# elasticdeeplearning/edl

Measured on AMD Instinct MI355X. Metric: img/s, higher is better.
Workload: dtype bf16; 1 GPU; model=resnet50_vd, global_batch=32, parallelism=dp1, graph_capture=True

## Files before the change

edl_amd/csrc/common.h:

```cpp
#pragma once
#include <hip/hip_runtime.h>
#include <hip/hip_bf16.h>

constexpr int kWave = 64;

static inline int elementwise_grid(long long n, int block) {
  long long want = (n + block - 1) / block;
  long long cap = 256LL * 8;
  return (int)(want < cap ? want : cap);
}

__device__ __forceinline__ int xcd_swizzle(int orig, int nwg) {
  const int nx = 8;
  const int q = nwg / nx, r = nwg % nx;
  const int xcd = orig % nx, local = orig / nx;
  return (xcd < r ? xcd * (q + 1) : r * (q + 1) + (xcd - r) * q) + local;
}

__device__ __forceinline__ float wave_reduce_sum(float v) {
#pragma unroll
  for (int off = 32; off > 0; off >>= 1) v += __shfl_down(v, off, 64);
  return v;
}

__device__ __forceinline__ float wave_reduce_max(float v) {
#pragma unroll
  for (int off = 32; off > 0; off >>= 1) v = fmaxf(v, __shfl_down(v, off, 64));
  return v;
}
```

edl_amd/csrc/fused_adam.hip:

```cpp
#include "common.h"
#include "launchers.h"

namespace {

struct AdamCoef {
  float lr, b1, b2, omb1, omb2, eps, scale, step_size, sqrt_bc2;
  bool decoupled;
};

__device__ __forceinline__ void adam_elem(const AdamCoef& c, const float wd,
                                          const float g, float& p, float& m,
                                          float& v) {
  float gs = c.scale * g;
  if (c.decoupled)
    p *= 1.0f - c.lr * wd;
  else
    gs = fmaf(wd, p, gs);
  m = fmaf(c.b1, m, c.omb1 * gs);
  v = fmaf(c.b2, v, (c.omb2 * gs) * gs);
  const float denom = sqrtf(v) / c.sqrt_bc2 + c.eps;
  p = fmaf(-c.step_size, m / denom, p);
}

__device__ __forceinline__ int adam_find_seg(const int* s_end, int lo,
                                             const int nseg, const int e) {
  int hi = nseg - 1;
  while (lo < hi) {
    const int mid = (lo + hi) >> 1;
    if (s_end[mid] > e) hi = mid; else lo = mid + 1;
  }
  return lo;
}

__device__ __forceinline__ int adam_next_seg(const int* s_end, int s,
                                             const int nseg, const int e) {
  while (s + 1 < nseg && e >= s_end[s]) ++s;
  return s;
}

}

extern "C" __global__ void fused_adam_f32(
    float* __restrict__ p, const float* __restrict__ g, float* __restrict__ m,
    float* __restrict__ v, const int* __restrict__ step_dev,
    const float* __restrict__ lr_dev, const float lr_host, const float b1,
    const float b2, const float omb1, const float omb2, const float ln_b1,
    const float ln_b2, const float eps, const float wd, const float scale,
    const int decoupled, const long long n, const int* __restrict__ seg_end,
    const float* __restrict__ seg_wd, const int nseg) {
  extern __shared__ int s_tab[];
  int* s_end = s_tab;
  float* s_wd = reinterpret_cast<float*>(s_tab + nseg);
  if (nseg > 0) {
    for (int k = threadIdx.x; k < nseg; k += blockDim.x) {
      s_end[k] = seg_end[k];
      s_wd[k] = seg_wd[k];
    }
    __syncthreads();
  }

  AdamCoef c;
  c.lr = lr_dev ? *lr_dev : lr_host;
  const int t = *step_dev;
  const float tf = (float)(t > 1 ? t : 1);
  c.b1 = b1; c.b2 = b2; c.omb1 = omb1; c.omb2 = omb2;
  c.eps = eps; c.scale = scale; c.decoupled = decoupled != 0;
  c.step_size = c.lr / -expm1f(tf * ln_b1);
  c.sqrt_bc2 = sqrtf(-expm1f(tf * ln_b2));

  const long long n4 = n >> 2;
  const float4* g4 = reinterpret_cast<const float4*>(g);
  float4* p4 = reinterpret_cast<float4*>(p);
  float4* m4 = reinterpret_cast<float4*>(m);
  float4* v4 = reinterpret_cast<float4*>(v);
  long long i = (long long)blockIdx.x * blockDim.x + threadIdx.x;
  const long long stride = (long long)gridDim.x * blockDim.x;
  int s = 0;
  for (; i < n4; i += stride) {
    float4 pg = g4[i], pp = p4[i], pm = m4[i], pv = v4[i];
    float w0 = wd, w1 = wd, w2 = wd, w3 = wd;
    if (nseg > 0) {
      const int e = (int)(i << 2);
      s = adam_find_seg(s_end, s, nseg, e);
      int q = s;
      w0 = s_wd[q];
      q = adam_next_seg(s_end, q, nseg, e + 1);
      w1 = s_wd[q];
      q = adam_next_seg(s_end, q, nseg, e + 2);
      w2 = s_wd[q];
      q = adam_next_seg(s_end, q, nseg, e + 3);
      w3 = s_wd[q];
    }
    adam_elem(c, w0, pg.x, pp.x, pm.x, pv.x);
    adam_elem(c, w1, pg.y, pp.y, pm.y, pv.y);
    adam_elem(c, w2, pg.z, pp.z, pm.z, pv.z);
    adam_elem(c, w3, pg.w, pp.w, pm.w, pv.w);
    m4[i] = pm;
    v4[i] = pv;
    p4[i] = pp;
  }
  for (long long j = (n4 << 2) + (long long)blockIdx.x * blockDim.x + threadIdx.x;
       j < n; j += stride) {
    float w = wd;
    if (nseg > 0) w = s_wd[adam_find_seg(s_end, 0, nseg, (int)j)];
    float pj = p[j], mj = m[j], vj = v[j];
    adam_elem(c, w, g[j], pj, mj, vj);
    m[j] = mj;
    v[j] = vj;
    p[j] = pj;
  }
}

extern "C" void launch_fused_adam_f32(
    float* p, const float* g, float* m, float* v, const int* step_dev,
    const float* lr_dev, float lr, float b1, float b2, float omb1, float omb2,
    float ln_b1, float ln_b2, float eps, float wd, float scale, int decoupled,
    long long n, const int* seg_end, const float* seg_wd, int nseg,
    hipStream_t stream) {
  const int block = 256;
  const int grid = elementwise_grid((n + 3) / 4, block);
  const size_t lds = (size_t)nseg * (sizeof(int) + sizeof(float));
  hipLaunchKernelGGL(fused_adam_f32, dim3(grid), dim3(block), lds, stream, p,
                     g, m, v, step_dev, lr_dev, lr, b1, b2, omb1, omb2, ln_b1,
                     ln_b2, eps, wd, scale, decoupled, n, seg_end, seg_wd,
                     nseg);
}
```

edl_amd/csrc/fused_sgd.hip:

```cpp
#include "common.h"
#include "launchers.h"

extern "C" __global__ void fused_sgd_f32(
    float* __restrict__ p, const float* __restrict__ g, float* __restrict__ m,
    const float lr_host, const float mu, const float wd, const float scale,
    const long long n, const float* __restrict__ lr_dev) {
  const float lr = lr_dev ? *lr_dev : lr_host;
  const long long n4 = n >> 2;
  const float4* g4 = reinterpret_cast<const float4*>(g);
  float4* p4 = reinterpret_cast<float4*>(p);
  float4* m4 = reinterpret_cast<float4*>(m);
  long long i = (long long)blockIdx.x * blockDim.x + threadIdx.x;
  const long long stride = (long long)gridDim.x * blockDim.x;
  for (; i < n4; i += stride) {
    float4 pg = g4[i], pp = p4[i], pm = m4[i];
    float d0 = fmaf(scale, pg.x, wd * pp.x);
    float d1 = fmaf(scale, pg.y, wd * pp.y);
    float d2 = fmaf(scale, pg.z, wd * pp.z);
    float d3 = fmaf(scale, pg.w, wd * pp.w);
    pm.x = fmaf(mu, pm.x, d0);
    pm.y = fmaf(mu, pm.y, d1);
    pm.z = fmaf(mu, pm.z, d2);
    pm.w = fmaf(mu, pm.w, d3);
    pp.x = fmaf(-lr, pm.x, pp.x);
    pp.y = fmaf(-lr, pm.y, pp.y);
    pp.z = fmaf(-lr, pm.z, pp.z);
    pp.w = fmaf(-lr, pm.w, pp.w);
    m4[i] = pm;
    p4[i] = pp;
  }
  for (long long j = (n4 << 2) + (long long)blockIdx.x * blockDim.x + threadIdx.x;
       j < n; j += stride) {
    float d = fmaf(scale, g[j], wd * p[j]);
    float mv = fmaf(mu, m[j], d);
    m[j] = mv;
    p[j] = fmaf(-lr, mv, p[j]);
  }
}

extern "C" void launch_fused_sgd_f32(float* p, const float* g, float* m,
                                     float lr, float mu, float wd, float scale,
                                     long long n, const float* lr_dev,
                                     hipStream_t stream) {
  const int block = 256;
  const int grid = elementwise_grid((n + 3) / 4, block);
  hipLaunchKernelGGL(fused_sgd_f32, dim3(grid), dim3(block), 0, stream,
                     p, g, m, lr, mu, wd, scale, n, lr_dev);
}
```

edl_amd/csrc/launchers.h:

```cpp
#pragma once
#include <hip/hip_runtime_api.h>

constexpr int kStatsPartRowCap = 192;

extern "C" {

void launch_fused_sgd_f32(float* p, const float* g, float* m, float lr,
                          float mu, float wd, float scale, long long n,
                          const float* lr_dev, hipStream_t stream);

constexpr int kAdamMaxSegments = 1024;
void launch_fused_adam_f32(float* p, const float* g, float* m, float* v,
                           const int* step_dev, const float* lr_dev, float lr,
                           float b1, float b2, float omb1, float omb2,
                           float ln_b1, float ln_b2, float eps, float wd,
                           float scale, int decoupled, long long n,
                           const int* seg_end, const float* seg_wd, int nseg,
                           hipStream_t stream);

void launch_kd_ce_fwd_f32(const float* s, const float* t, float* lpr, int B,
                          int C, hipStream_t stream);
void launch_kd_ce_bwd_f32(const float* s, const float* t, float* ds,
                          float gob, int B, int C, hipStream_t stream);
void launch_kd_ce_fwd_bf16(const void* s, const void* t, float* lpr, int B,
                           int C, hipStream_t stream);
void launch_kd_ce_bwd_bf16(const void* s, const void* t, void* ds, float gob,
                           int B, int C, hipStream_t stream);

void launch_softmax_ce_fwd(const void* s, int is_bf16, const long long* ya,
                           const long long* yb, const float* lam,
                           float* loss_row, float* lse, int* rank, float eps,
                           int B, int C, hipStream_t stream);
void launch_softmax_ce_bwd(const void* s, int is_bf16, const float* lse,
                           const long long* ya, const long long* yb,
                           const float* lam, const float* gout, void* ds,
                           float eps, float inv_B, int B, int C,
                           hipStream_t stream);

int bn_stats_grid(long long M, int C);
int bn_bwd_grid(long long M, int C);
void launch_bn_stats(const void* x, float* partial, int grid, long long M,
                     int C, hipStream_t s);
void launch_bn_finalize(float* partial, int nblocks, int zero_src,
                        const float* gamma, const float* beta, float* mean,
                        float* invstd, float* scale, float* shift,
                        float* rmean, float* rvar, float momentum, float eps,
                        long long M, int C, hipStream_t s);
void launch_bn_apply(const void* x, const void* res, void* y,
                     unsigned char* mask, const float* scale,
                     const float* shift, long long M, int C, bool relu,
                     bool add, hipStream_t s);
void launch_bn_apply_pad(const void* x, void* yp, unsigned char* mask,
                         const float* scale, const float* shift, int Nimg,
                         int H, int W, int C, hipStream_t s);
void launch_bn_bwd_reduce(const void* dy, const unsigned char* mask,
                          const void* x, const float* mean,
                          const float* invstd, float* partial, int grid,
                          long long M, int C, bool relu, hipStream_t s);
void launch_bn_bwd_finalize(const float* partial, int nblocks, float* sums,
                            int C, float* db_acc, float* dg_acc,
                            hipStream_t s);
void launch_bn_bwd_dx(const void* dy, const unsigned char* mask,
                      const void* x, const float* mean, const float* invstd,
                      const float* gamma, const float* sums, void* dx,
                      void* dres, long long M, int C, bool relu, bool add,
                      bool training, hipStream_t s);
void launch_bn_bwd_dx_pad(const void* dy, const unsigned char* mask,
                          const void* x, const float* mean,
                          const float* invstd, const float* gamma,
                          const float* sums, void* dxp, int Nimg, int H,
                          int W, int C, bool relu, hipStream_t s);
void launch_bn_bwd_fused(const void* dy, const unsigned char* mask,
                         const void* x, const float* mean,
                         const float* invstd, const float* gamma,
                         float* partial, float* sums, float* db_acc,
                         float* dg_acc, void* dx, void* dres, int* ws,
                         int grid, int nfin, long long M, int C, bool relu,
                         bool add, hipStream_t s);

int gemm_bt_tiles_m(int M, int N);
void launch_gemm_bt(const void* A, const void* B, void* C, int M, int N,
                    int K, float* bn_part, hipStream_t s);
void launch_gemm_bt_splitk(const void* A, const void* B, float* Cf32, int M,
                           int N, int K, int splitk, hipStream_t s);

int conv3x3_tiles_m(int M, int Cout);
int conv3x3_small_tiles_m(int M);
int conv3x3_pick_splitk(int M, int Cout, int Cin);
void launch_pad_nhwc(const void* x, void* xp, int Nimg, int H, int W, int Hp,
                     int Wp, int C, hipStream_t s);
void launch_pad_nhwc_cpad(const void* x, void* xp, int Nimg, int H, int W,
                          int Hp, int Wp, int Creal, int Cpad,
                          hipStream_t s);
void launch_conv3x3(const void* xp, const void* w3, void* y, int M, int Cout,
                    int Cin, int HW_out, int W_out, int Hp, int Wp,
                    int stride, float* cpart, int splitk, float* bn_part,
                    hipStream_t s);
void launch_conv3x3_grouped(const void* xp, const void* w3g, void* y, int M,
                            int Cout, int Cin, int HW_out, int W_out, int Hp,
                            int Wp, int stride, int gw, hipStream_t s);
void launch_conv3x3_small(const void* xp, const void* w3s, void* y, int M,
                          int Cout_real, int cpt, int HW_out, int W_out,
                          int Hp, int Wp, int stride, float* bn_part,
                          hipStream_t s);
void launch_conv3x3s2_dgrad(const void* dyp, const void* wcat, void* dx,
                            int Nimg, int H, int W, int Cin, int Cout,
                            int Hop, int Wop, hipStream_t s);

void launch_gemm_tn_splitk(const void* A, const void* B, float* C, int N1,
                           int N2, int K, int splitk, hipStream_t s);
void launch_gemm_tn3x3_splitk(const void* dy, const void* xpad, float* C,
                              int Cout, int Cin, int M, int Ho, int Wo,
                              int Hp, int Wp, int stride, int splitk,
                              int perm, hipStream_t s);
void launch_gemm_tn3x3_splitk_apad(const void* dyp, const void* xpad,
                                   float* C, int Cout, int Cin, int M, int Ho,
                                   int Wo, int Hp, int Wp, int stride,
                                   int splitk, int perm, hipStream_t s);
void launch_gemm_tn3x3_small(const void* dy, const void* xpad, float* C,
                             int N1v, int N2v, int M, int Ho, int Wo, int Hp,
                             int Wp, int CinP, int stride, int splitk,
                             hipStream_t s);

void launch_transpose_pad(const void* in, void* out, int M, int C, int Mp,
                          hipStream_t s);
void launch_shift9_transpose(const void* xp, void* out, int M, int C, int Mp,
                             int HW_out, int W_out, int Hp, int Wp,
                             int stride, hipStream_t s);
void launch_repack_dgrad_w3(const void* in, void* out, int Co, int Ci,
                            int mode, hipStream_t s);
void launch_cast_bf16_zero(float* src, void* dst, long long n, hipStream_t s);

void launch_maxpool3x3s2_fwd(const void* x, void* y, unsigned char* idx,
                             int N, int H, int W, int Ho, int Wo, int C,
                             hipStream_t s);
void launch_maxpool3x3s2_bwd(const void* dy, const unsigned char* idx,
                             void* dx, int N, int H, int W, int Ho, int Wo,
                             int C, hipStream_t s);

void launch_avgpool2x2_fwd(const void* x, void* y, int N, int H, int W,
                           int Ho, int Wo, int C, hipStream_t s);
void launch_avgpool2x2_bwd(const void* dy, void* dx, int N, int H, int W,
                           int Ho, int Wo, int C, hipStream_t s);

int dgc_workspace_words();
void launch_dgc_accumulate(const float* g, float* u, float* v,
                           const float* p, float mu, float wd, long long n,
                           unsigned* ws, int hist_copies, hipStream_t stream);
void launch_dgc_hist(const float* v, long long n, unsigned* ws, int pass,
                     hipStream_t stream);
void launch_dgc_pick(unsigned* ws, int pass, unsigned k, hipStream_t stream);
void launch_dgc_compact(float* v, float* u, long long n, int* payload,
                        unsigned k, unsigned* ws, hipStream_t stream);
void launch_dgc_scatter_add(float* out, long long n, const int* payload,
                            long long k, hipStream_t stream);

}
```

edl_amd/csrc/module.cpp:

```cpp
#include <iterator>
#include <mutex>
#include <unordered_map>
#include <unordered_set>
#include <torch/extension.h>

#include <c10/hip/HIPStream.h>
#include <hip/hip_runtime.h>

#include "launchers.h"

namespace {

hipStream_t cur_stream() {
  return c10::hip::getCurrentHIPStream().stream();
}


void check_nhwc_bf16(const torch::Tensor& x, const char* who, int cmod = 0) {
  TORCH_CHECK(x.is_cuda() && x.dim() == 4 &&
                  x.scalar_type() == torch::kBFloat16 &&
                  x.is_contiguous(torch::MemoryFormat::ChannelsLast),
              who, ": 4-D channels_last bf16 GPU tensor required");
  TORCH_CHECK(cmod <= 0 || x.size(1) % cmod == 0, who, ": C % ", cmod);
}

int out_extent(int64_t in, int64_t stride) {
  return (int)((in - 1) / stride + 1);
}

int64_t auto_splitk(int tiles, int64_t upper) {
  const int64_t sk = std::max<int64_t>(1, 512 / std::max(1, tiles));
  return std::min(sk, upper);
}

void check_bt_operands(const torch::Tensor& a, const torch::Tensor& b,
                       const char* who) {
  TORCH_CHECK(a.is_cuda() && b.is_cuda() && a.dim() == 2 && b.dim() == 2 &&
                  a.size(1) == b.size(1),
              who, ": [M,K] x [N,K] GPU tensors required");
  TORCH_CHECK(a.scalar_type() == torch::kBFloat16 &&
                  b.scalar_type() == torch::kBFloat16,
              who, ": bf16 only");
  TORCH_CHECK(a.size(1) % 64 == 0 && b.size(0) % 64 == 0, who,
              ": K,N % 64 == 0");
}

int tn_tiles(int n) { return n / (n % 128 == 0 ? 128 : 64); }

torch::Tensor out_or_zeros(const c10::optional<torch::Tensor>& out,
                           int64_t rows, int64_t cols,
                           torch::TensorOptions opts, const char* msg) {
  if (!out.has_value())
    return torch::zeros({rows, cols}, opts.dtype(torch::kFloat32));
  TORCH_CHECK(out->is_contiguous() &&
                  out->scalar_type() == torch::kFloat32 &&
                  out->numel() == rows * cols,
              msg);
  return *out;
}

float* acc_ptr(const c10::optional<torch::Tensor>& acc, int64_t C,
               const char* msg) {
  if (!acc.has_value()) return nullptr;
  TORCH_CHECK(acc->numel() == C && acc->is_contiguous() &&
                  acc->scalar_type() == torch::kFloat32,
              msg);
  return acc->data_ptr<float>();
}

struct PadNHW {
  int64_t n = 0, h = 0, w = 0;
};

PadNHW parse_pad_hw(const std::vector<int64_t>& pad_hw, long long M,
                    const char* who) {
  TORCH_CHECK(pad_hw.size() == 2, who, ": pad_hw = (H, W)");
  PadNHW p;
  p.h = pad_hw[0];
  p.w = pad_hw[1];
  TORCH_CHECK(p.h >= 1 && p.w >= 1 && M >= 1 && M % (p.h * p.w) == 0, who,
              ": pad_hw does not divide the rows of x");
  p.n = M / (p.h * p.w);
  TORCH_CHECK(p.n * (p.h + 2) * (p.w + 2) < (1LL << 31), who,
              ": padded pixel count must stay below 2^31");
  return p;
}

void dgc_check_flat(const torch::Tensor& t, const char* name) {
  TORCH_CHECK(t.is_cuda() && t.scalar_type() == torch::kFloat32 &&
                  t.dim() == 1 && t.is_contiguous(),
              "dgc: ", name, " must be a flat contiguous fp32 GPU tensor");
  TORCH_CHECK(t.numel() >= 1 && t.numel() < (1LL << 31),
              "dgc: 1 <= n < 2^31 required for ", name);
}

unsigned* dgc_ws_ptr(const torch::Tensor& ws, const torch::Tensor& like) {
  TORCH_CHECK(ws.is_cuda() && ws.device() == like.device() &&
                  ws.scalar_type() == torch::kInt32 && ws.is_contiguous() &&
                  ws.numel() == dgc_workspace_words(),
              "dgc: workspace must be the int32 GPU tensor of "
              "dgc_workspace_words() zeros");
  return reinterpret_cast<unsigned*>(ws.data_ptr<int>());
}

void dgc_check_k(int64_t k, const torch::Tensor& v) {
  TORCH_CHECK(k >= 1 && k <= v.numel(), "dgc: 1 <= k <= n required");
}

int* dgc_payload_ptr(const torch::Tensor& payload, int64_t k,
                     const torch::Tensor& like) {
  TORCH_CHECK(payload.is_cuda() && payload.device() == like.device() &&
                  payload.scalar_type() == torch::kInt32 &&
                  payload.is_contiguous() && payload.dim() == 2 &&
                  payload.size(0) == 2 && payload.size(1) == k,
              "dgc: payload must be a contiguous int32 [2, k] GPU tensor");
  return payload.data_ptr<int>();
}

void dgc_accumulate(torch::Tensor g, torch::Tensor u, torch::Tensor v,
                    c10::optional<torch::Tensor> p, double mu, double wd,
                    torch::Tensor ws, int64_t hist_copies) {
  dgc_check_flat(g, "g");
  dgc_check_flat(u, "u");
  dgc_check_flat(v, "v");
  TORCH_CHECK(g.numel() == u.numel() && g.numel() == v.numel() &&
                  g.device() == u.device() && g.device() == v.device(),
              "dgc: g, u, v must match in size and device");
  const float* pp = nullptr;
  if (p.has_value()) {
    dgc_check_flat(*p, "p");
    TORCH_CHECK(p->numel() == g.numel() && p->device() == g.device(),
                "dgc: p must match g");
    pp = p->data_ptr<float>();
  }
  TORCH_CHECK(hist_copies == 1 || hist_copies == 4, "dgc: hist_copies 1 or 4");
  launch_dgc_accumulate(g.data_ptr<float>(), u.data_ptr<float>(),
                        v.data_ptr<float>(), pp, (float)mu, (float)wd,
                        (long long)g.numel(), dgc_ws_ptr(ws, g),
                        (int)hist_copies, cur_stream());
}

void dgc_hist(torch::Tensor v, torch::Tensor ws, int64_t pass) {
  dgc_check_flat(v, "v");
  TORCH_CHECK(pass == 1 || pass == 2, "dgc_hist: pass 1 or 2");
  launch_dgc_hist(v.data_ptr<float>(), (long long)v.numel(),
                  dgc_ws_ptr(ws, v), (int)pass, cur_stream());
}

void dgc_pick(torch::Tensor v, torch::Tensor ws, int64_t pass, int64_t k) {
  dgc_check_flat(v, "v");
  dgc_check_k(k, v);
  TORCH_CHECK(pass >= 0 && pass <= 2, "dgc_pick: pass 0..2");
  launch_dgc_pick(dgc_ws_ptr(ws, v), (int)pass, (unsigned)k, cur_stream());
}

void dgc_compact(torch::Tensor v, torch::Tensor u, torch::Tensor payload,
                 torch::Tensor ws) {
  dgc_check_flat(v, "v");
  dgc_check_flat(u, "u");
  TORCH_CHECK(u.numel() == v.numel() && u.device() == v.device(),
              "dgc: u must match v");
  const int64_t k = payload.dim() == 2 ? payload.size(1) : -1;
  dgc_check_k(k, v);
  launch_dgc_compact(v.data_ptr<float>(), u.data_ptr<float>(),
                     (long long)v.numel(), dgc_payload_ptr(payload, k, v),
                     (unsigned)k, dgc_ws_ptr(ws, v), cur_stream());
}

void dgc_select(torch::Tensor v, torch::Tensor u, torch::Tensor payload,
                torch::Tensor ws) {
  const int64_t k = payload.dim() == 2 ? payload.size(1) : -1;
  dgc_pick(v, ws, 0, k);
  dgc_hist(v, ws, 1);
  dgc_pick(v, ws, 1, k);
  dgc_hist(v, ws, 2);
  dgc_pick(v, ws, 2, k);
  dgc_compact(v, u, payload, ws);
}

void dgc_scatter_add(torch::Tensor out, torch::Tensor payload) {
  dgc_check_flat(out, "out");
  const int64_t k = payload.dim() == 2 ? payload.size(1) : -1;
  TORCH_CHECK(k >= 1, "dgc: payload must be int32 [2, k]");
  launch_dgc_scatter_add(out.data_ptr<float>(), (long long)out.numel(),
                         dgc_payload_ptr(payload, k, out), (long long)k,
                         cur_stream());
}

void fused_sgd(torch::Tensor p, torch::Tensor g, torch::Tensor m, double lr,
               double momentum, double weight_decay, double grad_scale,
               c10::optional<torch::Tensor> lr_dev) {
  TORCH_CHECK(p.is_cuda() && g.is_cuda() && m.is_cuda(), "fused_sgd: GPU tensors required");
  TORCH_CHECK(p.scalar_type() == torch::kFloat32 && g.scalar_type() == torch::kFloat32 &&
                  m.scalar_type() == torch::kFloat32,
              "fused_sgd: fp32 only");
  TORCH_CHECK(p.is_contiguous() && g.is_contiguous() && m.is_contiguous(),
              "fused_sgd: contiguous flat buffers required");
  TORCH_CHECK(p.numel() == g.numel() && p.numel() == m.numel(), "fused_sgd: size mismatch");
  const float* lrp = nullptr;
  if (lr_dev.has_value()) {
    TORCH_CHECK(lr_dev->is_cuda() && lr_dev->scalar_type() == torch::kFloat32 &&
                    lr_dev->numel() == 1,
                "fused_sgd: lr_dev must be a fp32 GPU scalar");
    lrp = lr_dev->data_ptr<float>();
  }
  launch_fused_sgd_f32(p.data_ptr<float>(), g.data_ptr<float>(), m.data_ptr<float>(),
                       (float)lr, (float)momentum, (float)weight_decay,
                       (float)grad_scale, (long long)p.numel(), lrp, cur_stream());
}


struct AdamTableSeen {
  c10::weak_intrusive_ptr<c10::TensorImpl> impl;
  uint32_t version;
  long long n;
};

void adam_check_table(const torch::Tensor& seg_end, long long n) {
  static std::mutex mu;
  static std::unordered_map<const c10::TensorImpl*, AdamTableSeen> seen;
  std::lock_guard<std::mutex> lock(mu);
  const c10::TensorImpl* key = seg_end.unsafeGetTensorImpl();
  const uint32_t version = seg_end._version();
  auto it = seen.find(key);
  if (it != seen.end() && !it->second.impl.expired() &&
      it->second.version == version && it->second.n == n)
    return;
  hipStreamCaptureStatus cap = hipStreamCaptureStatusNone;
  TORCH_CHECK(hipStreamIsCapturing(cur_stream(), &cap) == hipSuccess,
              "fused_adam: hipStreamIsCapturing failed");
  if (cap != hipStreamCaptureStatusNone) return;
  auto host = seg_end.cpu();
  const int* e = host.data_ptr<int>();
  int prev = 0;
  for (int64_t k = 0; k < host.numel(); ++k) {
    TORCH_CHECK(e[k] >= prev, "fused_adam: seg_end must not decrease");
    prev = e[k];
  }
  TORCH_CHECK(prev == n, "fused_adam: last seg_end (", prev,
              ") must equal numel (", n, ")");
  for (auto e = seen.begin(); e != seen.end();)
    e = e->second.impl.expired() ? seen.erase(e) : std::next(e);
  seen.insert_or_assign(
      key, AdamTableSeen{c10::weak_intrusive_ptr<c10::TensorImpl>(
                             seg_end.getIntrusivePtr()),
                         version, n});
}

void fused_adam(torch::Tensor p, torch::Tensor g, torch::Tensor m,
                torch::Tensor v, torch::Tensor step_dev, double lr,
                double beta1, double beta2, double eps, double weight_decay,
                double grad_scale, bool decoupled,
                c10::optional<torch::Tensor> lr_dev,
                c10::optional<torch::Tensor> seg_end,
                c10::optional<torch::Tensor> seg_wd) {
  TORCH_CHECK(p.is_cuda() && g.is_cuda() && m.is_cuda() && v.is_cuda(),
              "fused_adam: GPU tensors required");
  TORCH_CHECK(p.scalar_type() == torch::kFloat32 &&
                  g.scalar_type() == torch::kFloat32 &&
                  m.scalar_type() == torch::kFloat32 &&
                  v.scalar_type() == torch::kFloat32,
              "fused_adam: fp32 only");
  TORCH_CHECK(p.is_contiguous() && g.is_contiguous() && m.is_contiguous() &&
                  v.is_contiguous(),
              "fused_adam: contiguous flat buffers required");
  const long long n = p.numel();
  TORCH_CHECK(g.numel() == n && m.numel() == n && v.numel() == n,
              "fused_adam: size mismatch");
  TORCH_CHECK(g.device() == p.device() && m.device() == p.device() &&
                  v.device() == p.device(),
              "fused_adam: p, g, m, v must share a device");
  for (const torch::Tensor* t : {&p, &g, &m, &v})
    TORCH_CHECK(reinterpret_cast<uintptr_t>(t->data_ptr()) % 16 == 0,
                "fused_adam: p, g, m, v must be 16-byte aligned (float4)");
  TORCH_CHECK(step_dev.is_cuda() && step_dev.device() == p.device() &&
                  step_dev.scalar_type() == torch::kInt32 &&
                  step_dev.numel() == 1,
              "fused_adam: step_dev must be an int32 GPU scalar");
  TORCH_CHECK(beta1 >= 0.0 && beta1 < 1.0 && beta2 >= 0.0 && beta2 < 1.0,
              "fused_adam: betas must lie in [0, 1)");
  const float* lrp = nullptr;
  if (lr_dev.has_value()) {
    TORCH_CHECK(lr_dev->is_cuda() && lr_dev->device() == p.device() &&
                    lr_dev->scalar_type() == torch::kFloat32 &&
                    lr_dev->numel() == 1,
                "fused_adam: lr_dev must be a fp32 GPU scalar");
    lrp = lr_dev->data_ptr<float>();
  }
  const int* endp = nullptr;
  const float* wdp = nullptr;
  int nseg = 0;
  TORCH_CHECK(seg_end.has_value() == seg_wd.has_value(),
              "fused_adam: seg_end and seg_wd come together");
  if (seg_end.has_value()) {
    TORCH_CHECK(seg_end->is_cuda() && seg_wd->is_cuda() &&
                    seg_end->device() == p.device() &&
                    seg_wd->device() == p.device() &&
                    seg_end->scalar_type() == torch::kInt32 &&
                    seg_wd->scalar_type() == torch::kFloat32 &&
                    seg_end->is_contiguous() && seg_wd->is_contiguous() &&
                    seg_end->dim() == 1 && seg_wd->dim() == 1,
                "fused_adam: seg_end int32 / seg_wd fp32 flat GPU tensors");
    TORCH_CHECK(seg_end->numel() == seg_wd->numel(),
                "fused_adam: seg_end and seg_wd differ in length");
    TORCH_CHECK(seg_end->numel() >= 1 &&
                    seg_end->numel() <= kAdamMaxSegments,
                "fused_adam: 1 <= segments <= ", kAdamMaxSegments,
                " per bucket (got ", seg_end->numel(), ")");
    TORCH_CHECK(n < (1LL << 31),
                "fused_adam: a segment table needs numel < 2^31");
    adam_check_table(*seg_end, n);
    endp = seg_end->data_ptr<int>();
    wdp = seg_wd->data_ptr<float>();
    nseg = (int)seg_end->numel();
  }
  if (n == 0) return;
  launch_fused_adam_f32(
      p.data_ptr<float>(), g.data_ptr<float>(), m.data_ptr<float>(),
      v.data_ptr<float>(), step_dev.data_ptr<int>(), lrp, (float)lr,
      (float)beta1, (float)beta2, (float)(1.0 - beta1), (float)(1.0 - beta2),
      (float)std::log(beta1), (float)std::log(beta2), (float)eps,
      (float)weight_decay, (float)grad_scale, decoupled ? 1 : 0, n, endp, wdp,
      nseg, cur_stream());
}

torch::Tensor kd_ce_forward(torch::Tensor s, torch::Tensor t) {
  TORCH_CHECK(s.is_cuda() && t.is_cuda(), "kd_ce: GPU tensors required");
  TORCH_CHECK(s.dim() == 2 && t.sizes() == s.sizes(), "kd_ce: [B,C] logits expected");
  TORCH_CHECK(s.scalar_type() == t.scalar_type(), "kd_ce: dtype mismatch");
  auto sc = s.contiguous();
  auto tc = t.contiguous();
  const int B = (int)s.size(0), C = (int)s.size(1);
  auto lpr = torch::empty({B}, s.options().dtype(torch::kFloat32));
  if (s.scalar_type() == torch::kFloat32) {
    launch_kd_ce_fwd_f32(sc.data_ptr<float>(), tc.data_ptr<float>(),
                         lpr.data_ptr<float>(), B, C, cur_stream());
  } else if (s.scalar_type() == torch::kBFloat16) {
    launch_kd_ce_fwd_bf16(sc.data_ptr(), tc.data_ptr(), lpr.data_ptr<float>(), B, C,
                          cur_stream());
  } else {
    TORCH_CHECK(false, "kd_ce: fp32/bf16 only");
  }
  return lpr;
}

torch::Tensor kd_ce_backward(torch::Tensor s, torch::Tensor t, double gout_over_B) {
  auto sc = s.contiguous();
  auto tc = t.contiguous();
  const int B = (int)s.size(0), C = (int)s.size(1);
  auto ds = torch::empty_like(sc);
  if (s.scalar_type() == torch::kFloat32) {
    launch_kd_ce_bwd_f32(sc.data_ptr<float>(), tc.data_ptr<float>(), ds.data_ptr<float>(),
                         (float)gout_over_B, B, C, cur_stream());
  } else if (s.scalar_type() == torch::kBFloat16) {
    launch_kd_ce_bwd_bf16(sc.data_ptr(), tc.data_ptr(), ds.data_ptr(),
                          (float)gout_over_B, B, C, cur_stream());
  } else {
    TORCH_CHECK(false, "kd_ce: fp32/bf16 only");
  }
  return ds;
}

std::pair<const long long*, const float*> check_softmax_ce_inputs(
    const torch::Tensor& s, const torch::Tensor& ya,
    const c10::optional<torch::Tensor>& yb,
    const c10::optional<torch::Tensor>& lam) {
  TORCH_CHECK(s.is_cuda() && ya.device() == s.device(),
              "softmax_ce: logits and labels on one GPU required");
  TORCH_CHECK(s.dim() == 2 && s.size(0) >= 1 && s.size(1) >= 1,
              "softmax_ce: [B,C] logits expected");
  TORCH_CHECK(s.scalar_type() == torch::kFloat32 ||
                  s.scalar_type() == torch::kBFloat16,
              "softmax_ce: fp32/bf16 only");
  TORCH_CHECK(s.is_contiguous(), "softmax_ce: contiguous logits required");
  TORCH_CHECK(s.numel() < (1LL << 31), "softmax_ce: B*C < 2^31");
  const int64_t B = s.size(0);
  TORCH_CHECK(ya.scalar_type() == torch::kInt64 && ya.dim() == 1 &&
                  ya.numel() == B && ya.is_contiguous(),
              "softmax_ce: labels must be contiguous int64 [B]");
  TORCH_CHECK(yb.has_value() == lam.has_value(),
              "softmax_ce: labels_b and lam go together");
  if (!yb.has_value()) return {nullptr, nullptr};
  TORCH_CHECK(yb->is_cuda() && yb->scalar_type() == torch::kInt64 &&
                  yb->dim() == 1 && yb->numel() == B && yb->is_contiguous(),
              "softmax_ce: labels_b must be contiguous int64 [B] on the GPU");
  TORCH_CHECK(lam->is_cuda() && lam->scalar_type() == torch::kFloat32 &&
                  lam->dim() == 1 && lam->numel() == B && lam->is_contiguous(),
              "softmax_ce: lam must be contiguous fp32 [B] on the GPU");
  return {(const long long*)yb->data_ptr<int64_t>(), lam->data_ptr<float>()};
}

std::vector<torch::Tensor> softmax_ce_forward(torch::Tensor s, torch::Tensor ya,
                                              c10::optional<torch::Tensor> yb,
                                              c10::optional<torch::Tensor> lam,
                                              double eps) {
  auto mix = check_softmax_ce_inputs(s, ya, yb, lam);
  const int B = (int)s.size(0), C = (int)s.size(1);
  auto opts = s.options().dtype(torch::kFloat32);
  auto loss_row = torch::empty({B}, opts);
  auto lse = torch::empty({B}, opts);
  auto rank = torch::empty({B}, s.options().dtype(torch::kInt32));
  launch_softmax_ce_fwd(s.data_ptr(), s.scalar_type() == torch::kBFloat16,
                        (const long long*)ya.data_ptr<int64_t>(), mix.first,
                        mix.second, loss_row.data_ptr<float>(),
                        lse.data_ptr<float>(), rank.data_ptr<int>(), (float)eps,
                        B, C, cur_stream());
  return {loss_row, lse, rank};
}

torch::Tensor softmax_ce_backward(torch::Tensor s, torch::Tensor lse,
                                  torch::Tensor ya,
                                  c10::optional<torch::Tensor> yb,
                                  c10::optional<torch::Tensor> lam, double eps,
                                  torch::Tensor gout, double inv_B) {
  auto mix = check_softmax_ce_inputs(s, ya, yb, lam);
  const int B = (int)s.size(0), C = (int)s.size(1);
  TORCH_CHECK(lse.is_cuda() && lse.scalar_type() == torch::kFloat32 &&
                  lse.numel() == B && lse.is_contiguous(),
              "softmax_ce: lse must be contiguous fp32 [B] on the GPU");
  TORCH_CHECK(gout.is_cuda() && gout.scalar_type() == torch::kFloat32 &&
                  gout.numel() == 1,
              "softmax_ce: gout must be a fp32 GPU scalar");
  auto ds = torch::empty_like(s);
  launch_softmax_ce_bwd(s.data_ptr(), s.scalar_type() == torch::kBFloat16,
                        lse.data_ptr<float>(),
                        (const long long*)ya.data_ptr<int64_t>(), mix.first,
                        mix.second, gout.data_ptr<float>(), ds.data_ptr(),
                        (float)eps, (float)inv_B, B, C, cur_stream());
  return ds;
}

static std::unordered_set<const void*>& pooled_ptr_set() {
  static std::unordered_set<const void*> ptrs;
  return ptrs;
}

static torch::Tensor part_pool_get(int rows, int64_t cols,
                                   torch::TensorOptions opts) {
  static std::unordered_map<int64_t, torch::Tensor> pool;
  const int64_t key = ((int64_t)opts.device().index() << 48) |
                      ((int64_t)rows << 28) | cols;
  auto it = pool.find(key);
  if (it != pool.end()) return it->second;
  auto t = torch::zeros({rows, cols}, opts);
  pool.emplace(key, t);
  pooled_ptr_set().insert(t.data_ptr());
  return t;
}

torch::Tensor stats_part_buf(int tiles_m, int64_t cols,
                             torch::TensorOptions opts) {
  opts = opts.dtype(torch::kFloat32);
  const int rows = std::min(tiles_m, kStatsPartRowCap);
  return tiles_m > rows ? part_pool_get(rows, cols, opts)
                        : torch::empty({rows, cols}, opts);
}

void check_bn_inputs_eval(const torch::Tensor& x, int64_t C) {
  TORCH_CHECK(x.is_cuda() && x.scalar_type() == torch::kBFloat16,
              "bn: bf16 GPU tensor required");
  TORCH_CHECK(C % 8 == 0, "bn: C % 8 == 0 required, got ", C);
}

void check_bn_inputs(const torch::Tensor& x, int64_t C) {
  check_bn_inputs_eval(x, C);
  TORCH_CHECK(C <= 2048, "bn: C <= 2048 supported");
  TORCH_CHECK((C & (C - 1)) == 0,
              "bn: training needs a power-of-two C (8..2048): the stats and "
              "reduce kernels split each 256-thread block into C/8-thread "
              "rows; got ", C);
}

std::vector<torch::Tensor> bn_fwd_train(torch::Tensor x, torch::Tensor gamma,
                                        torch::Tensor beta, torch::Tensor rmean,
                                        torch::Tensor rvar, double momentum,
                                        double eps,
                                        c10::optional<torch::Tensor> res,
                                        bool relu,
                                        c10::optional<torch::Tensor> pre_part,
                                        c10::optional<std::vector<int64_t>> pad_hw) {
  const int64_t C = gamma.numel();
  TORCH_CHECK(x.dim() == 2 && x.size(1) == C && x.is_contiguous(),
              "bn: x must be a contiguous [M, C] view");
  check_bn_inputs(x, C);
  const long long M = x.numel() / C;
  PadNHW pad;
  if (pad_hw.has_value()) {
    TORCH_CHECK(relu && !res.has_value(),
                "bn: pad_hw needs relu and no residual");
    pad = parse_pad_hw(*pad_hw, M, "bn");
  }
  auto opts = gamma.options().dtype(torch::kFloat32);
  const int grid = bn_stats_grid(M, (int)C);
  auto partial = torch::empty({grid, 2 * C}, opts);
  auto mean = torch::empty({C}, opts);
  auto invstd = torch::empty({C}, opts);
  auto scale = torch::empty({C}, opts);
  auto shift = torch::empty({C}, opts);
  auto y = pad.n ? torch::empty({pad.n, pad.h + 2, pad.w + 2, C}, x.options())
                 : torch::empty_like(x);
  auto msk = relu ? torch::empty({M, C / 8}, x.options().dtype(torch::kUInt8))
                  : torch::empty({0}, x.options().dtype(torch::kUInt8));
  auto s = cur_stream();
  int fin_grid = grid;
  if (pre_part.has_value()) {
    TORCH_CHECK(pre_part->is_contiguous() &&
                    pre_part->scalar_type() == torch::kFloat32 &&
                    pre_part->dim() == 2 && pre_part->size(1) == 2 * C,
                "bn: pre_part [tiles, 2C] fp32");
    partial = *pre_part;
    fin_grid = (int)pre_part->size(0);
  } else {
    launch_bn_stats(x.data_ptr(), partial.data_ptr<float>(), grid, M, (int)C,
                    s);
  }
  const int zero_src =
      pre_part.has_value() &&
      pooled_ptr_set().count((const void*)partial.data_ptr());
  launch_bn_finalize(partial.data_ptr<float>(), fin_grid,
                     zero_src, gamma.data_ptr<float>(),
                     beta.data_ptr<float>(), mean.data_ptr<float>(),
                     invstd.data_ptr<float>(), scale.data_ptr<float>(),
                     shift.data_ptr<float>(),
                     rmean.defined() ? rmean.data_ptr<float>() : nullptr,
                     rvar.defined() ? rvar.data_ptr<float>() : nullptr,
                     (float)momentum, (float)eps, M, (int)C, s);
  if (pad.n) {
    launch_bn_apply_pad(x.data_ptr(), y.data_ptr(),
                        (unsigned char*)msk.data_ptr(),
                        scale.data_ptr<float>(), shift.data_ptr<float>(),
                        (int)pad.n, (int)pad.h, (int)pad.w, (int)C, s);
  } else {
    launch_bn_apply(x.data_ptr(), res.has_value() ? res->data_ptr() : nullptr,
                    y.data_ptr(),
                    relu ? (unsigned char*)msk.data_ptr() : nullptr,
                    scale.data_ptr<float>(), shift.data_ptr<float>(), M,
                    (int)C, relu, res.has_value(), s);
  }
  return {y, mean, invstd, msk};
}

torch::Tensor bn_fwd_eval(torch::Tensor x, torch::Tensor scale, torch::Tensor shift,
                          c10::optional<torch::Tensor> res, bool relu) {
  const int64_t C = scale.numel();
  check_bn_inputs_eval(x, C);
  const long long M = x.numel() / C;
  auto y = torch::empty_like(x);
  launch_bn_apply(x.data_ptr(), res.has_value() ? res->data_ptr() : nullptr,
                  y.data_ptr(), nullptr,
                  scale.data_ptr<float>(), shift.data_ptr<float>(),
                  M, (int)C, relu, res.has_value(), cur_stream());
  return y;
}

std::vector<torch::Tensor> bn_bwd(torch::Tensor dy, c10::optional<torch::Tensor> msk,
                                  torch::Tensor x,
                                  torch::Tensor mean, torch::Tensor invstd,
                                  torch::Tensor gamma, bool relu, bool add,
                                  bool training,
                                  c10::optional<torch::Tensor> dgamma_acc,
                                  c10::optional<torch::Tensor> dbeta_acc,
                                  c10::optional<std::vector<int64_t>> pad_hw) {
  const int64_t C = gamma.numel();
  check_bn_inputs(x, C);
  const long long M = x.numel() / C;
  auto opts = gamma.options().dtype(torch::kFloat32);
  const int grid = bn_bwd_grid(M, (int)C);
  auto sums = torch::empty({2, C}, opts);
  const char* fenv = getenv("EDL_BN_BWD_FUSED");
  const bool fused_bwd = fenv ? atoi(fenv) != 0 : false;
  PadNHW pad;
  if (pad_hw.has_value() && !(fused_bwd && training)) {
    TORCH_CHECK(training && !add, "bn_bwd: pad_hw needs training, no residual");
    pad = parse_pad_hw(*pad_hw, M, "bn_bwd");
  }
  auto dx = pad.n ? torch::empty({pad.n, pad.h + 2, pad.w + 2, C}, x.options())
                  : torch::empty_like(x);
  auto dres = add ? torch::empty_like(x) : torch::Tensor();
  auto s = cur_stream();
  auto dyc = dy.is_contiguous() ? dy : dy.contiguous();
  TORCH_CHECK(!relu || (msk.has_value() && msk->numel() == M * (C / 8)),
              "bn_bwd: relu path needs the fwd mask");
  const unsigned char* mp =
      relu ? (const unsigned char*)msk->data_ptr() : nullptr;
  float* dg_acc = acc_ptr(dgamma_acc, C, "bn_bwd: dgamma_acc fp32 [C]");
  float* db_acc = acc_ptr(dbeta_acc, C, "bn_bwd: dbeta_acc fp32 [C]");
  if (fused_bwd && training) {
    static std::unordered_map<int, torch::Tensor> ws_pool;
    const int dev = (int)x.device().index();
    auto wit = ws_pool.find(dev);
    if (wit == ws_pool.end())
      wit = ws_pool.emplace(dev, torch::zeros({4},
          x.options().dtype(torch::kInt32))).first;
    const long long total8 = M * (C / 8);
    int fgrid = (int)((total8 + 1023) / 1024);
    if (fgrid < grid) fgrid = grid;
    if (fgrid > 512) fgrid = 512;
    int nfin = (int)(2 * C) / 256;
    if (nfin < 1) nfin = 1;
    if (nfin > 8) nfin = 8;
    auto fpartial = torch::empty({fgrid, 2 * C}, opts);
    launch_bn_bwd_fused(dyc.data_ptr(), mp, x.data_ptr(),
                        mean.data_ptr<float>(), invstd.data_ptr<float>(),
                        gamma.data_ptr<float>(), fpartial.data_ptr<float>(),
                        sums.data_ptr<float>(), db_acc, dg_acc, dx.data_ptr(),
                        add ? dres.data_ptr() : nullptr,
                        wit->second.data_ptr<int>(), fgrid, nfin, M, (int)C,
                        relu, add, s);
    return {dx, sums[1], sums[0], dres};
  }
  auto partial = torch::empty({grid, 2 * C}, opts);
  launch_bn_bwd_reduce(dyc.data_ptr(), mp, x.data_ptr(),
                       mean.data_ptr<float>(), invstd.data_ptr<float>(),
                       partial.data_ptr<float>(), grid, M, (int)C, relu, s);
  launch_bn_bwd_finalize(partial.data_ptr<float>(), grid, sums.data_ptr<float>(),
                         (int)C, db_acc, dg_acc, s);
  if (pad.n) {
    launch_bn_bwd_dx_pad(dyc.data_ptr(), mp, x.data_ptr(),
                         mean.data_ptr<float>(), invstd.data_ptr<float>(),
                         gamma.data_ptr<float>(), sums.data_ptr<float>(),
                         dx.data_ptr(), (int)pad.n, (int)pad.h, (int)pad.w,
                         (int)C, relu, s);
  } else {
    launch_bn_bwd_dx(dyc.data_ptr(), mp, x.data_ptr(), mean.data_ptr<float>(),
                     invstd.data_ptr<float>(), gamma.data_ptr<float>(),
                     sums.data_ptr<float>(), dx.data_ptr(),
                     add ? dres.data_ptr() : nullptr, M, (int)C, relu, add,
                     training, s);
  }
  return {dx, sums[1], sums[0], dres};
}

std::vector<torch::Tensor> gemm_bt_impl(const torch::Tensor& a,
                                        const torch::Tensor& b,
                                        bool with_stats) {
  check_bt_operands(a, b, "gemm_bt");
  auto ac = a.contiguous();
  auto bc = b.contiguous();
  const int M = (int)a.size(0), K = (int)a.size(1), N = (int)b.size(0);
  auto c = torch::empty({M, N}, a.options());
  torch::Tensor part;
  if (with_stats)
    part = stats_part_buf(gemm_bt_tiles_m(M, N), 2 * N, a.options());
  launch_gemm_bt(ac.data_ptr(), bc.data_ptr(), c.data_ptr(), M, N, K,
                 with_stats ? part.data_ptr<float>() : nullptr, cur_stream());
  return {c, part};
}

torch::Tensor gemm_bt(torch::Tensor a, torch::Tensor b) {
  return gemm_bt_impl(a, b, false)[0];
}

std::vector<torch::Tensor> gemm_bt_stats(torch::Tensor a, torch::Tensor b) {
  return gemm_bt_impl(a, b, true);
}

torch::Tensor pad_nhwc_flat(const torch::Tensor& x, int cpad, hipStream_t s) {
  const int Nimg = (int)x.size(0), C = (int)x.size(1);
  const int H = (int)x.size(2), W = (int)x.size(3);
  const int Hp = H + 2, Wp = W + 2;
  auto xp = torch::empty({(long long)Nimg * Hp * Wp * cpad}, x.options());
  if (C == cpad) {
    launch_pad_nhwc(x.data_ptr(), xp.data_ptr(), Nimg, H, W, Hp, Wp, C, s);
  } else {
    launch_pad_nhwc_cpad(x.data_ptr(), xp.data_ptr(), Nimg, H, W, Hp, Wp, C,
                         cpad, s);
  }
  return xp;
}

torch::Tensor conv3x3_grouped_fwd(torch::Tensor x, torch::Tensor w3g,
                                  int64_t stride) {
  check_nhwc_bf16(x, "conv3x3g");
  const int Nimg = (int)x.size(0), Cin = (int)x.size(1);
  const int H = (int)x.size(2), W = (int)x.size(3);
  const int Cout = (int)w3g.size(0);
  TORCH_CHECK(w3g.size(1) % 9 == 0 && w3g.is_contiguous(), "conv3x3g: w3g");
  const int gw = (int)(w3g.size(1) / 9);
  TORCH_CHECK(gw % 64 == 0 && Cin % gw == 0, "conv3x3g: gw % 64, Cin % gw");
  TORCH_CHECK(Cin % 64 == 0 && Cout % 64 == 0 && Cin == Cout,
              "conv3x3g: C % 64, equal in/out");
  const int Hout = out_extent(H, stride), Wout = out_extent(W, stride);
  const long long M = (long long)Nimg * Hout * Wout;
  auto s = cur_stream();
  auto xp = pad_nhwc_flat(x, Cin, s);
  auto y = torch::empty({M, Cout}, x.options());
  launch_conv3x3_grouped(xp.data_ptr(), w3g.data_ptr(), y.data_ptr(), (int)M,
                         Cout, Cin, Hout * Wout, Wout, H + 2, W + 2,
                         (int)stride, gw, s);
  return y;
}

std::vector<torch::Tensor> conv3x3_small_impl(const torch::Tensor& x,
                                              const torch::Tensor& w3s,
                                              int64_t cout_real, int64_t cpt,
                                              int64_t stride,
                                              bool with_stats) {
  check_nhwc_bf16(x, "conv3x3s");
  TORCH_CHECK(stride == 1 || stride == 2, "conv3x3s: stride 1 or 2");
  TORCH_CHECK(cpt == 16 || cpt == 32 || cpt == 64, "conv3x3s: cpt 16/32/64");
  const int Nimg = (int)x.size(0), Cin = (int)x.size(1);
  const int H = (int)x.size(2), W = (int)x.size(3);
  TORCH_CHECK(Cin <= cpt, "conv3x3s: Cin <= cpt");
  const int taps_pad = cpt == 16 ? 12 : (cpt == 32 ? 10 : 9);
  TORCH_CHECK(w3s.is_contiguous() && w3s.size(0) == 64 &&
                  w3s.size(1) == taps_pad * cpt,
              "conv3x3s: w3s [64, taps_pad*cpt]");
  TORCH_CHECK(cout_real >= 1 && cout_real <= 64, "conv3x3s: cout <= 64");
  const int Hout = out_extent(H, stride), Wout = out_extent(W, stride);
  const long long M = (long long)Nimg * Hout * Wout;
  auto s = cur_stream();
  auto xp = pad_nhwc_flat(x, (int)cpt, s);
  auto y = torch::empty({M, cout_real}, x.options());
  torch::Tensor bpart;
  if (with_stats)
    bpart = stats_part_buf(conv3x3_small_tiles_m((int)M), 2 * cout_real,
                           x.options());
  launch_conv3x3_small(xp.data_ptr(), w3s.data_ptr(), y.data_ptr(), (int)M,
                       (int)cout_real, (int)cpt, Hout * Wout, Wout, H + 2,
                       W + 2, (int)stride,
                       with_stats ? bpart.data_ptr<float>() : nullptr, s);
  return {y, bpart};
}

torch::Tensor conv3x3_small_fwd(torch::Tensor x, torch::Tensor w3s,
                                int64_t cout_real, int64_t cpt,
                                int64_t stride) {
  return conv3x3_small_impl(x, w3s, cout_real, cpt, stride, false)[0];
}

std::vector<torch::Tensor> conv3x3_small_fwd_stats(torch::Tensor x,
                                                   torch::Tensor w3s,
                                                   int64_t cout_real,
                                                   int64_t cpt,
                                                   int64_t stride) {
  return conv3x3_small_impl(x, w3s, cout_real, cpt, stride, true);
}


torch::Tensor pad_nhwc(torch::Tensor x) {
  check_nhwc_bf16(x, "pad_nhwc", 8);
  const int Nimg = (int)x.size(0), C = (int)x.size(1);
  const int H = (int)x.size(2), W = (int)x.size(3);
  auto xp = torch::empty({Nimg, H + 2, W + 2, C}, x.options());
  launch_pad_nhwc(x.data_ptr(), xp.data_ptr(), Nimg, H, W, H + 2, W + 2, C,
                  cur_stream());
  return xp;
}

void check_padded(const torch::Tensor& xp, int64_t H, int64_t W,
                  const char* who) {
  TORCH_CHECK(xp.is_cuda() && xp.dim() == 4 &&
                  xp.scalar_type() == torch::kBFloat16 && xp.is_contiguous(),
              who, ": xp must be a contiguous [N, H+2, W+2, C] bf16 buffer");
  TORCH_CHECK(H >= 1 && W >= 1 && xp.size(1) == H + 2 && xp.size(2) == W + 2,
              who, ": xp is not the padded layout of an H x W image");
}

torch::Tensor conv3x3s2_dgrad_padded(torch::Tensor dyp, torch::Tensor wcat,
                                     int64_t H, int64_t W) {
  const int64_t Ho = (H + 1) / 2, Wo = (W + 1) / 2;
  check_padded(dyp, Ho, Wo, "s2dgrad");
  const int Nimg = (int)dyp.size(0), Cout = (int)dyp.size(3);
  const int Cin = (int)(wcat.size(0));
  TORCH_CHECK(wcat.is_contiguous() && wcat.size(1) == 9 * Cout,
              "s2dgrad: wcat [Cin, 9*Cout]");
  TORCH_CHECK(Cin % 64 == 0 && Cout % 64 == 0, "s2dgrad: C % 64");
  auto dx = torch::empty({(long long)Nimg * H * W, Cin}, dyp.options());
  launch_conv3x3s2_dgrad(dyp.data_ptr(), wcat.data_ptr(), dx.data_ptr(), Nimg,
                         (int)H, (int)W, Cin, Cout, (int)Ho + 2, (int)Wo + 2,
                         cur_stream());
  return dx;
}

torch::Tensor conv3x3s2_dgrad(torch::Tensor dy, torch::Tensor wcat,
                              int64_t H, int64_t W) {
  check_nhwc_bf16(dy, "s2dgrad dy", 64);
  TORCH_CHECK((H + 1) / 2 == dy.size(2) && (W + 1) / 2 == dy.size(3),
              "s2dgrad: shape");
  return conv3x3s2_dgrad_padded(pad_nhwc(dy), wcat, H, W);
}

torch::Tensor repack_dgrad_w3(torch::Tensor w_smaj, int64_t ci,
                              int64_t mode) {
  TORCH_CHECK(w_smaj.is_cuda() && w_smaj.scalar_type() == torch::kBFloat16 &&
                  w_smaj.is_contiguous() && w_smaj.dim() == 2 &&
                  w_smaj.size(1) == 9 * ci,
              "repack_dgrad_w3: [Co, 9*Ci] bf16");
  const int Co = (int)w_smaj.size(0);
  TORCH_CHECK(Co % 64 == 0 && ci % 64 == 0, "repack_dgrad_w3: C % 64");
  auto out = torch::empty({ci, (long long)9 * Co}, w_smaj.options());
  launch_repack_dgrad_w3(w_smaj.data_ptr(), out.data_ptr(), Co, (int)ci,
                         (int)mode, cur_stream());
  return out;
}

std::vector<torch::Tensor> maxpool3x3s2_fwd(torch::Tensor x) {
  check_nhwc_bf16(x, "maxpool3x3s2", 8);
  const int N = (int)x.size(0), C = (int)x.size(1);
  const int H = (int)x.size(2), W = (int)x.size(3);
  const int Ho = (H + 1) / 2, Wo = (W + 1) / 2;
  auto y = torch::empty({N, C, Ho, Wo},
                        x.options().memory_format(torch::MemoryFormat::ChannelsLast));
  auto idx = torch::empty({(long long)N * Ho * Wo * C},
                          x.options().dtype(torch::kUInt8));
  launch_maxpool3x3s2_fwd(x.data_ptr(), y.data_ptr(),
                          idx.data_ptr<unsigned char>(), N, H, W, Ho, Wo, C,
                          cur_stream());
  return {y, idx};
}

torch::Tensor maxpool3x3s2_bwd(torch::Tensor dy, torch::Tensor idx,
                               int64_t H, int64_t W) {
  check_nhwc_bf16(dy, "maxpool3x3s2_bwd");
  const int N = (int)dy.size(0), C = (int)dy.size(1);
  const int Ho = (int)dy.size(2), Wo = (int)dy.size(3);
  auto dx = torch::empty({N, C, (long long)H, (long long)W},
                         dy.options().memory_format(torch::MemoryFormat::ChannelsLast));
  launch_maxpool3x3s2_bwd(dy.data_ptr(), idx.data_ptr<unsigned char>(),
                          dx.data_ptr(), N, (int)H, (int)W, Ho, Wo, C,
                          cur_stream());
  return dx;
}

torch::Tensor avgpool2x2_fwd(torch::Tensor x) {
  check_nhwc_bf16(x, "avgpool2x2", 8);
  const int N = (int)x.size(0), C = (int)x.size(1);
  const int H = (int)x.size(2), W = (int)x.size(3);
  const int Ho = (H + 1) / 2, Wo = (W + 1) / 2;
  auto y = torch::empty({N, C, Ho, Wo},
                        x.options().memory_format(torch::MemoryFormat::ChannelsLast));
  launch_avgpool2x2_fwd(x.data_ptr(), y.data_ptr(), N, H, W, Ho, Wo, C,
                        cur_stream());
  return y;
}

torch::Tensor avgpool2x2_bwd(torch::Tensor dy, int64_t H, int64_t W) {
  const int N = (int)dy.size(0), C = (int)dy.size(1);
  const int Ho = (int)dy.size(2), Wo = (int)dy.size(3);
  auto dyc = dy.contiguous(torch::MemoryFormat::ChannelsLast);
  auto dx = torch::empty({N, C, H, W},
                         dy.options().memory_format(torch::MemoryFormat::ChannelsLast));
  launch_avgpool2x2_bwd(dyc.data_ptr(), dx.data_ptr(), N, (int)H, (int)W, Ho,
                        Wo, C, cur_stream());
  return dx;
}

torch::Tensor conv3x3_wgrad_operand_padded(torch::Tensor xp, int64_t H,
                                           int64_t W, int64_t stride) {
  check_padded(xp, H, W, "wgrad_operand");
  TORCH_CHECK(stride == 1 || stride == 2, "wgrad_operand: stride 1 or 2");
  const int Nimg = (int)xp.size(0), Cin = (int)xp.size(3);
  const int Hp = (int)H + 2, Wp = (int)W + 2;
  const int Hout = out_extent(H, stride), Wout = out_extent(W, stride);
  const int M = Nimg * Hout * Wout;
  const int Mp = (M + 63) / 64 * 64;
  auto out = torch::empty({(long long)9 * Cin, Mp}, xp.options());
  launch_shift9_transpose(xp.data_ptr(), out.data_ptr(), M, Cin, Mp,
                          Hout * Wout, Wout, Hp, Wp, (int)stride,
                          cur_stream());
  return out;
}

torch::Tensor conv3x3_wgrad_operand(torch::Tensor x, int64_t stride) {
  auto xp = pad_nhwc(x);
  return conv3x3_wgrad_operand_padded(xp, x.size(2), x.size(3), stride);
}

torch::Tensor gemm_bt_splitk(torch::Tensor a, torch::Tensor b, int64_t splitk) {
  check_bt_operands(a, b, "gemm_bt_splitk");
  auto ac = a.contiguous();
  auto bc = b.contiguous();
  const int M = (int)a.size(0), K = (int)a.size(1), N = (int)b.size(0);
  if (splitk <= 0) {
    const int tiles = ((M + 127) / 128) * ((N + 63) / 64);
    splitk = auto_splitk(tiles, K / 64);
  }
  auto c = torch::zeros({M, N}, a.options().dtype(torch::kFloat32));
  launch_gemm_bt_splitk(ac.data_ptr(), bc.data_ptr(), c.data_ptr<float>(), M, N,
                        K, (int)splitk, cur_stream());
  return c;
}

torch::Tensor gemm_tn_splitk(torch::Tensor a, torch::Tensor b, int64_t splitk,
                             c10::optional<torch::Tensor> out) {
  TORCH_CHECK(a.is_cuda() && b.is_cuda() && a.dim() == 2 && b.dim() == 2 &&
                  a.size(0) == b.size(0),
              "gemm_tn_splitk: [K,N1] x [K,N2] GPU");
  TORCH_CHECK(a.scalar_type() == torch::kBFloat16 &&
                  b.scalar_type() == torch::kBFloat16,
              "gemm_tn_splitk: bf16 only");
  auto ac = a.contiguous();
  auto bc = b.contiguous();
  const int K = (int)a.size(0), N1 = (int)a.size(1), N2 = (int)b.size(1);
  TORCH_CHECK(N1 % 64 == 0 && N2 % 64 == 0, "gemm_tn_splitk: N1,N2 % 64");
  const int nchunks = (K + 63) / 64;
  if (splitk <= 0) splitk = auto_splitk(tn_tiles(N1) * tn_tiles(N2), nchunks);
  splitk = std::min<int64_t>(splitk, nchunks);
  auto c = out_or_zeros(out, N1, N2, a.options(),
                        "gemm_tn_splitk: out fp32 contiguous [N1,N2]");
  launch_gemm_tn_splitk(ac.data_ptr(), bc.data_ptr(), c.data_ptr<float>(), N1,
                        N2, K, (int)splitk, cur_stream());
  return c;
}

torch::Tensor gemm_tn3x3_splitk_padded(torch::Tensor dy, torch::Tensor xp,
                                       int64_t H64, int64_t W64,
                                       int64_t stride, int64_t splitk,
                                       c10::optional<torch::Tensor> out) {
  check_padded(xp, H64, W64, "gemm_tn3x3");
  TORCH_CHECK(stride == 1 || stride == 2, "gemm_tn3x3: stride 1 or 2");
  const bool dy_padded = dy.dim() == 4;
  TORCH_CHECK(dy.is_cuda() && (dy.dim() == 2 || dy_padded) &&
                  dy.scalar_type() == torch::kBFloat16,
              "gemm_tn3x3: dy [M,Cout] or padded [N,Ho+2,Wo+2,Cout] bf16");
  const int Nimg = (int)xp.size(0), Cin = (int)xp.size(3);
  const int H = (int)H64, W = (int)W64;
  const int Hp = H + 2, Wp = W + 2;
  const int Ho = out_extent(H, stride), Wo = out_extent(W, stride);
  const int M = Nimg * Ho * Wo;
  const int Cout = (int)dy.size(dy_padded ? 3 : 1);
  if (dy_padded) {
    check_padded(dy, Ho, Wo, "gemm_tn3x3 dy");
    TORCH_CHECK(dy.size(0) == Nimg, "gemm_tn3x3: dy batch != xp batch");
  } else {
    TORCH_CHECK((int)dy.size(0) == M, "gemm_tn3x3: dy2d rows != N*Ho*Wo");
  }
  TORCH_CHECK(Cin % 64 == 0 && Cout % 64 == 0, "gemm_tn3x3: C % 64");
  auto dyc = dy.contiguous();
  auto s = cur_stream();
  const int nchunks = (M + 63) / 64;
  if (splitk <= 0)
    splitk = auto_splitk(tn_tiles(Cout) * 9 * tn_tiles(Cin), nchunks);
  splitk = std::min<int64_t>(splitk, nchunks);
  auto c = out_or_zeros(out, Cout, 9 * Cin, xp.options(),
                        "gemm_tn3x3_splitk: out fp32 contiguous");
  const int perm = (c.dim() == 2 && c.size(1) == 9 * Cin) ? 0 : Cin;
  if (dy_padded)
    launch_gemm_tn3x3_splitk_apad(dyc.data_ptr(), xp.data_ptr(),
                                  c.data_ptr<float>(), Cout, Cin, M, Ho, Wo,
                                  Hp, Wp, (int)stride, (int)splitk, perm, s);
  else
    launch_gemm_tn3x3_splitk(dyc.data_ptr(), xp.data_ptr(),
                             c.data_ptr<float>(), Cout, Cin, M, Ho, Wo, Hp, Wp,
                             (int)stride, (int)splitk, perm, s);
  return c;
}

torch::Tensor gemm_tn3x3_splitk(torch::Tensor dy2d, torch::Tensor x,
                                int64_t stride, int64_t splitk,
                                c10::optional<torch::Tensor> out) {
  TORCH_CHECK(dy2d.dim() == 2, "gemm_tn3x3: dy2d [M,Cout] bf16");
  auto xp = pad_nhwc(x);
  return gemm_tn3x3_splitk_padded(dy2d, xp, x.size(2), x.size(3), stride,
                                  splitk, out);
}

torch::Tensor transpose_pad(torch::Tensor x) {
  TORCH_CHECK(x.is_cuda() && x.dim() == 2 &&
                  x.scalar_type() == torch::kBFloat16 && x.is_contiguous(),
              "transpose_pad: contiguous 2-D bf16 GPU tensor");
  const int M = (int)x.size(0), C = (int)x.size(1);
  TORCH_CHECK(C % 8 == 0, "transpose_pad: C % 8");
  const int Mp = (M + 63) / 64 * 64;
  auto y = torch::empty({C, Mp}, x.options());
  launch_transpose_pad(x.data_ptr(), y.data_ptr(), M, C, Mp, cur_stream());
  return y;
}

struct Conv3x3Geom {
  int Cin, Cout, Hp, Wp, Hout, Wout;
  long long M;
};

Conv3x3Geom conv3x3_geom(const torch::Tensor& xp, const torch::Tensor& w3,
                         int64_t stride, int64_t H, int64_t W) {
  check_padded(xp, H, W, "conv3x3");
  TORCH_CHECK(stride == 1 || stride == 2, "conv3x3: stride 1 or 2");
  Conv3x3Geom g;
  g.Cin = (int)xp.size(3);
  g.Cout = (int)w3.size(0);
  TORCH_CHECK(w3.size(1) == 9 * g.Cin && w3.is_contiguous(),
              "conv3x3: w3 shape");
  TORCH_CHECK(g.Cin % 64 == 0 && g.Cout % 64 == 0, "conv3x3: C % 64");
  g.Hp = (int)H + 2;
  g.Wp = (int)W + 2;
  g.Hout = out_extent(H, stride);
  g.Wout = out_extent(W, stride);
  g.M = (long long)xp.size(0) * g.Hout * g.Wout;
  return g;
}

std::vector<torch::Tensor> conv3x3_fwd_impl(const torch::Tensor& xp,
                                            const torch::Tensor& w3,
                                            int64_t stride, int64_t H,
                                            int64_t W, bool with_stats) {
  const Conv3x3Geom g = conv3x3_geom(xp, w3, stride, H, W);
  const int M = (int)g.M;
  auto s = cur_stream();
  const int splitk = conv3x3_pick_splitk(M, g.Cout, g.Cin);
  torch::Tensor y, bpart;
  if (splitk > 1) {
    auto part =
        part_pool_get(M, g.Cout, xp.options().dtype(torch::kFloat32));
    launch_conv3x3(xp.data_ptr(), w3.data_ptr(), nullptr, M, g.Cout, g.Cin,
                   g.Hout * g.Wout, g.Wout, g.Hp, g.Wp, (int)stride,
                   part.data_ptr<float>(), splitk, nullptr, s);
    y = torch::empty({g.M, g.Cout}, xp.options());
    launch_cast_bf16_zero(part.data_ptr<float>(), y.data_ptr(),
                          g.M * g.Cout, s);
  } else {
    y = torch::empty({g.M, g.Cout}, xp.options());
    if (with_stats)
      bpart = stats_part_buf(conv3x3_tiles_m(M, g.Cout), 2 * g.Cout,
                             xp.options());
    launch_conv3x3(xp.data_ptr(), w3.data_ptr(), y.data_ptr(), M, g.Cout,
                   g.Cin, g.Hout * g.Wout, g.Wout, g.Hp, g.Wp, (int)stride,
                   nullptr, 1, with_stats ? bpart.data_ptr<float>() : nullptr,
                   s);
  }
  return {y, bpart};
}

torch::Tensor conv3x3_fwd_padded(torch::Tensor xp, torch::Tensor w3,
                                 int64_t stride, int64_t H, int64_t W) {
  return conv3x3_fwd_impl(xp, w3, stride, H, W, false)[0];
}

std::vector<torch::Tensor> conv3x3_fwd_stats_padded(torch::Tensor xp,
                                                    torch::Tensor w3,
                                                    int64_t stride, int64_t H,
                                                    int64_t W) {
  return conv3x3_fwd_impl(xp, w3, stride, H, W, true);
}

torch::Tensor conv3x3_fwd(torch::Tensor x, torch::Tensor w3, int64_t stride) {
  check_nhwc_bf16(x, "conv3x3", 64);
  return conv3x3_fwd_padded(pad_nhwc(x), w3, stride, x.size(2), x.size(3));
}

std::vector<torch::Tensor> conv3x3_fwd_stats(torch::Tensor x, torch::Tensor w3,
                                             int64_t stride) {
  check_nhwc_bf16(x, "conv3x3", 64);
  return conv3x3_fwd_stats_padded(pad_nhwc(x), w3, stride, x.size(2),
                                  x.size(3));
}

torch::Tensor gemm_tn3x3_small(torch::Tensor dy2d, torch::Tensor x,
                               int64_t stride, int64_t splitk) {
  check_nhwc_bf16(x, "tn3x3s");
  TORCH_CHECK(stride == 1 || stride == 2, "tn3x3s: stride 1 or 2");
  const int Nimg = (int)x.size(0), Cin = (int)x.size(1);
  const int H = (int)x.size(2), W = (int)x.size(3);
  TORCH_CHECK(Cin >= 1 && Cin <= 64, "tn3x3s: Cin <= 64");
  const int Hout = out_extent(H, stride), Wout = out_extent(W, stride);
  const long long M = (long long)Nimg * Hout * Wout;
  TORCH_CHECK(dy2d.is_cuda() && dy2d.is_contiguous() && dy2d.dim() == 2 &&
                  dy2d.scalar_type() == torch::kBFloat16 &&
                  dy2d.size(0) == M && dy2d.size(1) == 64,
              "tn3x3s: dy2d [M, 64] bf16");
  int CinP = 8;
  while (CinP < Cin) CinP <<= 1;
  const int N2 = 9 * CinP;
  const int N2v = (N2 + 63) / 64 * 64;
  auto s = cur_stream();
  auto xp = pad_nhwc_flat(x, CinP, s);
  if (splitk <= 0) {
    const int nch = (int)((M + 63) / 64);
    splitk = auto_splitk(N2v / 64, std::max(1, nch));
  }
  auto c = torch::zeros({64, N2v}, x.options().dtype(torch::kFloat32));
  launch_gemm_tn3x3_small(dy2d.data_ptr(), xp.data_ptr(), c.data_ptr<float>(),
                          64, N2v, (int)M, Hout, Wout, H + 2, W + 2, CinP,
                          (int)stride, (int)splitk, s);
  return c;
}

}

PYBIND11_MODULE(TORCH_EXTENSION_NAME, m) {
  m.def("fused_sgd", &fused_sgd,
        "fused flat momentum-SGD update (p,g,m flat fp32; folds grad_scale)",
        py::arg("p"), py::arg("g"), py::arg("m"), py::arg("lr"),
        py::arg("momentum"), py::arg("weight_decay"), py::arg("grad_scale"),
        py::arg("lr_dev") = py::none());
  m.def("fused_adam", &fused_adam,
        "fused flat Adam/AdamW update (p,g,m,v flat fp32; step count and lr "
        "read from device scalars; optional per-segment decay table of at "
        "most 1024 segments); does not advance step_dev",
        py::arg("p"), py::arg("g"), py::arg("m"), py::arg("v"),
        py::arg("step_dev"), py::arg("lr"), py::arg("beta1"),
        py::arg("beta2"), py::arg("eps"), py::arg("weight_decay"),
        py::arg("grad_scale"), py::arg("decoupled"),
        py::arg("lr_dev") = py::none(), py::arg("seg_end") = py::none(),
        py::arg("seg_wd") = py::none());
  m.attr("ADAM_MAX_SEGMENTS") = kAdamMaxSegments;
  m.def("dgc_workspace_words", &dgc_workspace_words,
        "int32 words of the (zero-initialised) DGC select workspace");
  m.def("dgc_accumulate", &dgc_accumulate,
        "DGC: u = mu*u + (g + wd*p); v += u; radix-select pass 0 histogram",
        py::arg("g"), py::arg("u"), py::arg("v"), py::arg("p"), py::arg("mu"),
        py::arg("wd"), py::arg("ws"), py::arg("hist_copies") = 4);
  m.def("dgc_hist", &dgc_hist, "DGC radix-select histogram pass 1 or 2",
        py::arg("v"), py::arg("ws"), py::arg("pass_"));
  m.def("dgc_pick", &dgc_pick, "DGC radix-select: fix one digit (pass 0..2)",
        py::arg("v"), py::arg("ws"), py::arg("pass_"), py::arg("k"));
  m.def("dgc_compact", &dgc_compact,
        "DGC: write the selected (idx, bits) into payload [2,k]; zero v, u",
        py::arg("v"), py::arg("u"), py::arg("payload"), py::arg("ws"));
  m.def("dgc_select", &dgc_select,
        "DGC: pick 0, (hist, pick) x 2 and compact, after dgc_accumulate",
        py::arg("v"), py::arg("u"), py::arg("payload"), py::arg("ws"));
  m.def("dgc_scatter_add", &dgc_scatter_add,
        "DGC decode: out[idx] += val for one rank's payload",
        py::arg("out"), py::arg("payload"));
  m.def("kd_ce_forward", &kd_ce_forward, "KD soft-label CE forward -> per-row loss");
  m.def("kd_ce_backward", &kd_ce_backward, "KD soft-label CE backward -> dlogits");
  m.def("softmax_ce_forward", &softmax_ce_forward,
        "hard-label CE (label smoothing, optional mixup) fwd -> "
        "(loss_row, lse, rank)",
        py::arg("s"), py::arg("labels"), py::arg("labels_b") = py::none(),
        py::arg("lam") = py::none(), py::arg("eps") = 0.0);
  m.def("softmax_ce_backward", &softmax_ce_backward,
        "hard-label CE bwd -> dlogits (gout is a device scalar)",
        py::arg("s"), py::arg("lse"), py::arg("labels"), py::arg("labels_b"),
        py::arg("lam"), py::arg("eps"), py::arg("gout"), py::arg("inv_B"));
  m.def("bn_fwd_train", &bn_fwd_train,
        "fused NHWC bf16 BN(+add)+ReLU train fwd -> (y, mean, invstd, mask)",
        py::arg("x"), py::arg("gamma"), py::arg("beta"), py::arg("rmean"),
        py::arg("rvar"), py::arg("momentum"), py::arg("eps"), py::arg("res"),
        py::arg("relu"), py::arg("pre_part") = py::none(),
        py::arg("pad_hw") = py::none());
  m.def("bn_fwd_eval", &bn_fwd_eval, "fused NHWC bf16 BN(+add)+ReLU eval fwd");
  m.def("bn_bwd", &bn_bwd,
        "fused BN(+add)+ReLU bwd -> (dx, dgamma, dbeta, dres?)",
        py::arg("dy"), py::arg("msk"), py::arg("x"), py::arg("mean"),
        py::arg("invstd"), py::arg("gamma"), py::arg("relu"), py::arg("add"),
        py::arg("training"), py::arg("dgamma_acc") = py::none(),
        py::arg("dbeta_acc") = py::none(), py::arg("pad_hw") = py::none());
  m.def("pad_nhwc", &pad_nhwc,
        "channels_last bf16 [N,C,H,W] -> zero-halo padded [N,H+2,W+2,C]");
  m.def("conv3x3_fwd_padded", &conv3x3_fwd_padded,
        "conv3x3_fwd on an already padded xp [N,H+2,W+2,Cin]", py::arg("xp"),
        py::arg("w3"), py::arg("stride"), py::arg("H"), py::arg("W"));
  m.def("conv3x3_fwd_stats_padded", &conv3x3_fwd_stats_padded,
        "conv3x3_fwd_stats on an already padded xp", py::arg("xp"),
        py::arg("w3"), py::arg("stride"), py::arg("H"), py::arg("W"));
  m.def("conv3x3s2_dgrad_padded", &conv3x3s2_dgrad_padded,
        "conv3x3s2_dgrad on an already padded dy [N,Ho+2,Wo+2,Cout]",
        py::arg("dyp"), py::arg("wcat"), py::arg("H"), py::arg("W"));
  m.def("gemm_tn3x3_splitk_padded", &gemm_tn3x3_splitk_padded,
        "gemm_tn3x3_splitk on padded xp; dy [M,Cout] or padded 4-D",
        py::arg("dy"), py::arg("xp"), py::arg("H"), py::arg("W"),
        py::arg("stride"), py::arg("splitk") = 0, py::arg("out") = py::none());
  m.def("conv3x3_wgrad_operand_padded", &conv3x3_wgrad_operand_padded,
        "conv3x3_wgrad_operand on an already padded xp", py::arg("xp"),
        py::arg("H"), py::arg("W"), py::arg("stride"));
  m.def("gemm_bt", &gemm_bt, "bf16 MFMA GEMM: C[M,N] = A[M,K] @ B[N,K]^T");
  m.def("conv3x3_fwd", &conv3x3_fwd,
        "implicit-GEMM 3x3 same-pad conv (stride 1/2) -> y2d [M, Cout]");
  m.def("conv3x3_fwd_stats", &conv3x3_fwd_stats,
        "conv3x3_fwd + BN stats partials -> (y2d, part-or-None)");
  m.def("gemm_bt_stats", &gemm_bt_stats,
        "gemm_bt + BN stats partials -> (C, part)");
  m.def("transpose_pad", &transpose_pad,
        "bf16 [M,C] -> [C, ceil64(M)] transpose with zero pad");
  m.def("gemm_bt_splitk", &gemm_bt_splitk,
        "split-K bt GEMM -> fp32 C (wgrad shapes)", py::arg("a"), py::arg("b"),
        py::arg("splitk") = 0);
  m.def("gemm_tn3x3_splitk", &gemm_tn3x3_splitk,
        "direct conv3x3 wgrad: fp32 dW3[Cout,9Cin] = dY^T @ gather3x3(pad(x))",
        py::arg("dy2d"), py::arg("x"), py::arg("stride"), py::arg("splitk") = 0,
        py::arg("out") = py::none());
  m.def("gemm_tn3x3_small", &gemm_tn3x3_small, py::arg("dy2d"),
        py::arg("x"), py::arg("stride"), py::arg("splitk") = 0,
        "stem wgrad: dY^T @ gather3x3(cpad(x)) -> fp32 [64, N2v] (G3S)");
  m.def("gemm_tn_splitk", &gemm_tn_splitk,
        "split-K TN GEMM: fp32 C[N1,N2] = A[K,N1]^T @ B[K,N2] (direct wgrad)",
        py::arg("a"), py::arg("b"), py::arg("splitk") = 0,
        py::arg("out") = py::none());
  m.def("conv3x3_wgrad_operand", &conv3x3_wgrad_operand,
        "padded shifted transpose of conv3x3 input -> [9*Cin, Mp]");
  m.def("avgpool2x2_fwd", &avgpool2x2_fwd, "2x2/s2 ceil avg pool (NHWC bf16)");
  m.def("conv3x3_grouped_fwd", &conv3x3_grouped_fwd,
        "grouped (16ch/group) 3x3 conv fwd -> y2d [M, Cout]");
  m.def("conv3x3s2_dgrad", &conv3x3s2_dgrad,
        "stride-2 3x3 same-pad dgrad (parity implicit GEMM) -> dx2d [N*H*W, Cin]");
  m.def("conv3x3_small_fwd", &conv3x3_small_fwd,
        "small-channel 3x3 conv (deep stem) -> y2d [M, cout_real]");
  m.def("conv3x3_small_fwd_stats", &conv3x3_small_fwd_stats,
        "stem conv + BN stats partials -> (y2d, part)");
  m.def("repack_dgrad_w3", &repack_dgrad_w3,
        "dgrad weight repack [Co,9Ci]->[Ci,9Co] (mode 0 rot / 1 s2 order)");
  m.def("maxpool3x3s2_fwd", &maxpool3x3s2_fwd,
        "3x3/s2/p1 max pool NHWC bf16 -> (y, tap idx)");
  m.def("maxpool3x3s2_bwd", &maxpool3x3s2_bwd,
        "3x3/s2/p1 max pool backward (bounded gather via tap idx)");
  m.def("avgpool2x2_bwd", &avgpool2x2_bwd, "2x2/s2 ceil avg pool backward");
  m.attr("_arch") = "gfx950";
}
```

edl_amd/csrc/transpose.hip:

```cpp
#include "common.h"
#include "launchers.h"

using bf16 = __hip_bfloat16;

extern "C" __global__ void transpose_pad_kernel(
    const bf16* __restrict__ in, bf16* __restrict__ out, const int M,
    const int C, const int Mp) {
  __shared__ bf16 tile[64][64 + 4];
  const int tm0 = blockIdx.x * 64;
  const int tc0 = blockIdx.y * 64;
  const int lr = threadIdx.x >> 3;
  const int lc = (threadIdx.x & 7) * 8;
  for (int half = 0; half < 2; ++half) {
    const int m = tm0 + half * 32 + lr;
    if (m < M && tc0 + lc < C) {
      const bf16* src = in + (long long)m * C + tc0 + lc;
      *reinterpret_cast<uint4*>(&tile[half * 32 + lr][lc]) =
          *reinterpret_cast<const uint4*>(__builtin_assume_aligned(src, 16));
    } else {
      uint4 z = {0, 0, 0, 0};
      *reinterpret_cast<uint4*>(&tile[half * 32 + lr][lc]) = z;
    }
  }
  __syncthreads();
  for (int half = 0; half < 2; ++half) {
    const int c = tc0 + half * 32 + lr;
    if (c < C) {
      bf16 v[8];
#pragma unroll
      for (int i = 0; i < 8; ++i) v[i] = tile[lc + i][half * 32 + lr];
      bf16* dst = out + (long long)c * Mp + tm0 + lc;
      *reinterpret_cast<uint4*>(__builtin_assume_aligned(dst, 16)) = *reinterpret_cast<const uint4*>(v);
    }
  }
}

extern "C" void launch_transpose_pad(const void* in, void* out, int M, int C,
                                     int Mp, hipStream_t s) {
  dim3 grid((Mp + 63) / 64, (C + 63) / 64);
  hipLaunchKernelGGL(transpose_pad_kernel, grid, dim3(256), 0, s,
                     (const bf16*)in, (bf16*)out, M, C, Mp);
}

extern "C" __global__ void shift9_transpose_kernel(
    const bf16* __restrict__ xp, bf16* __restrict__ out, const int M,
    const int C, const int Mp, const int HW_out, const int W_out, const int Hp,
    const int Wp, const int stride_hw) {
  __shared__ bf16 tile[64][64 + 4];
  const int s = blockIdx.z;
  const int shift = ((s / 3) * Wp + (s % 3)) * C;
  const int tm0 = blockIdx.x * 64;
  const int tc0 = blockIdx.y * 64;
  const int lr = threadIdx.x >> 3;
  const int lc = (threadIdx.x & 7) * 8;
  for (int half = 0; half < 2; ++half) {
    const int m = tm0 + half * 32 + lr;
    uint4 v = {0, 0, 0, 0};
    if (m < M && tc0 + lc < C) {
      const int n_img = m / HW_out;
      const int rem = m % HW_out;
      const int h = rem / W_out, w = rem % W_out;
      const long long prow =
          ((long long)n_img * Hp + h * stride_hw) * Wp + w * stride_hw;
      v = *reinterpret_cast<const uint4*>(
          __builtin_assume_aligned(xp + prow * C + shift + tc0 + lc, 16));
    }
    *reinterpret_cast<uint4*>(&tile[half * 32 + lr][lc]) = v;
  }
  __syncthreads();
  for (int half = 0; half < 2; ++half) {
    const int c = tc0 + half * 32 + lr;
    if (c < C) {
      bf16 v[8];
#pragma unroll
      for (int i = 0; i < 8; ++i) v[i] = tile[lc + i][half * 32 + lr];
      bf16* dst = out + ((long long)s * C + c) * Mp + tm0 + lc;
      *reinterpret_cast<uint4*>(__builtin_assume_aligned(dst, 16)) = *reinterpret_cast<const uint4*>(v);
    }
  }
}

extern "C" void launch_shift9_transpose(const void* xp, void* out, int M, int C,
                                        int Mp, int HW_out, int W_out, int Hp,
                                        int Wp, int stride, hipStream_t s) {
  dim3 grid((Mp + 63) / 64, (C + 63) / 64, 9);
  hipLaunchKernelGGL(shift9_transpose_kernel, grid, dim3(256), 0, s,
                     (const bf16*)xp, (bf16*)out, M, C, Mp, HW_out, W_out, Hp,
                     Wp, stride);
}

__constant__ int S2D_ORDER[9] = {4, 3, 5, 1, 7, 0, 2, 6, 8};

extern "C" __global__ void repack_dgrad_w3_kernel(
    const __hip_bfloat16* __restrict__ in, __hip_bfloat16* __restrict__ out,
    const int Co, const int Ci, const int mode) {
  __shared__ __hip_bfloat16 tile[64][64 + 8];
  const int s = blockIdx.y;
  const int tap = mode == 0 ? 8 - s : S2D_ORDER[s];
  const int tiles_co = Co >> 6;
  const int ci0 = (blockIdx.x / tiles_co) << 6;
  const int co0 = (blockIdx.x % tiles_co) << 6;
  const int lane = threadIdx.x & 63;
  const int quad = threadIdx.x >> 6;
  {
    const int c8 = lane & 7;
    const int rr = (lane >> 3) + quad * 8;
    for (int half = 0; half < 2; ++half) {
      const int r = rr + half * 32;
      const __hip_bfloat16* src =
          in + ((long long)(co0 + r) * 9 + tap) * Ci + ci0 + c8 * 8;
      *reinterpret_cast<uint4*>(
          __builtin_assume_aligned(&tile[r][c8 * 8], 16)) =
          *reinterpret_cast<const uint4*>(__builtin_assume_aligned(src, 16));
    }
  }
  __syncthreads();
  {
    const int c8 = lane & 7;
    const int rr = (lane >> 3) + quad * 8;
    for (int half = 0; half < 2; ++half) {
      const int r = rr + half * 32;
      __hip_bfloat16* dst =
          out + ((long long)(ci0 + r) * 9 + s) * Co + co0 + c8 * 8;
      uint4 v;
      __hip_bfloat16* pv = reinterpret_cast<__hip_bfloat16*>(&v);
#pragma unroll
      for (int k = 0; k < 8; ++k) pv[k] = tile[c8 * 8 + k][r];
      *reinterpret_cast<uint4*>(__builtin_assume_aligned(dst, 16)) = v;
    }
  }
}

extern "C" void launch_repack_dgrad_w3(const void* in, void* out, int Co,
                                       int Ci, int mode, hipStream_t s) {
  const dim3 grid((Ci >> 6) * (Co >> 6), 9);
  hipLaunchKernelGGL(repack_dgrad_w3_kernel, grid, dim3(256), 0, s,
                     (const __hip_bfloat16*)in, (__hip_bfloat16*)out, Co, Ci,
                     mode);
}

extern "C" __global__ void cast_bf16_zero_kernel(
    float* __restrict__ src, __hip_bfloat16* __restrict__ dst,
    const long long n4) {
  typedef __hip_bfloat16 bf16;
  long long i = (long long)blockIdx.x * blockDim.x + threadIdx.x;
  const long long stride = (long long)gridDim.x * blockDim.x;
  const float4 z = {0.0f, 0.0f, 0.0f, 0.0f};
  for (; i < n4; i += stride) {
    float4* ps = reinterpret_cast<float4*>(
        __builtin_assume_aligned(src + i * 4, 16));
    const float4 v = *ps;
    ulong1 packed;
    bf16* pv = reinterpret_cast<bf16*>(&packed);
    pv[0] = __float2bfloat16(v.x);
    pv[1] = __float2bfloat16(v.y);
    pv[2] = __float2bfloat16(v.z);
    pv[3] = __float2bfloat16(v.w);
    *reinterpret_cast<ulong1*>(__builtin_assume_aligned(dst + i * 4, 8)) =
        packed;
    *ps = z;
  }
}

extern "C" void launch_cast_bf16_zero(float* src, void* dst, long long n,
                                      hipStream_t s) {
  const long long n4 = n / 4;
  int grid = (int)((n4 + 255) / 256);
  if (grid > 4096) grid = 4096;
  hipLaunchKernelGGL(cast_bf16_zero_kernel, dim3(grid), dim3(256), 0, s, src,
                     (__hip_bfloat16*)dst, n4);
}
```

edl_amd/ops/adam.py:

```python
import torch

from . import ext
from ..train.bucketed_ddp import _view_like

ADAM_MAX_SEGMENTS = 1024


class FusedAdam:
    handles_grad_scale = True

    def __init__(self, params, lr=1e-3, betas=(0.9, 0.999), eps=1e-8,
                 weight_decay=0.0, decoupled=False, no_decay=None,
                 grad_scale=1.0, reducer=None):
        betas = (float(betas[0]), float(betas[1]))
        if not (0.0 <= betas[0] < 1.0 and 0.0 <= betas[1] < 1.0):
            raise ValueError("FusedAdam: betas must lie in [0, 1)")
        if eps < 0.0 or lr < 0.0 or weight_decay < 0.0:
            raise ValueError("FusedAdam: lr, eps, weight_decay must be >= 0")
        self._all_params = list(params)
        self._index = {id(p): i for i, p in enumerate(self._all_params)}
        if no_decay is None:
            nd = []
        elif callable(no_decay):
            nd = [i for i, p in enumerate(self._all_params) if no_decay(p)]
        else:
            ids = {id(p) for p in no_decay}
            nd = [i for i, p in enumerate(self._all_params) if id(p) in ids]
        self._no_decay = set(nd)
        self.defaults = dict(lr=float(lr), betas=betas, eps=float(eps),
                             weight_decay=float(weight_decay), amsgrad=False,
                             decoupled=bool(decoupled), no_decay=sorted(nd))
        self.param_groups = [dict(
            self.defaults,
            params=[p for p in self._all_params if p.requires_grad])]
        self.grad_scale = grad_scale
        self._reducer = reducer
        self._buckets = None
        self._step_t = None
        self._lr_dev = None
        if reducer is not None:
            self.attach(reducer)

    def attach(self, reducer):
        self._reducer = reducer
        self._buckets = None
        reducer._attached_opt = self
        return self

    def set_lr(self, lr):
        for g in self.param_groups:
            g["lr"] = float(lr)
        if self._lr_dev is not None:
            self._lr_dev.fill_(float(lr))

    @property
    def step_count(self):
        return 0 if self._step_t is None else int(self._step_t.item())

    def _param_wd(self, p):
        wd = self.param_groups[0]["weight_decay"]
        return 0.0 if self._index.get(id(p)) in self._no_decay else wd

    def _build_tables(self):
        for bk in self._buckets:
            segs = []
            for (off, n), p in zip(bk["offsets"], bk["params"]):
                wd = self._param_wd(p)
                if segs and segs[-1][1] == wd:
                    segs[-1][0] = off + n
                else:
                    segs.append([off + n, wd])
            bk["segs"] = segs
            bk["wd"] = segs[0][1] if len(segs) == 1 else 0.0
            bk["seg_end"] = bk["seg_wd"] = None
            if len(segs) > 1 and bk["p"].is_cuda:
                if len(segs) > ADAM_MAX_SEGMENTS:
                    raise RuntimeError(
                        "FusedAdam: a bucket alternates decay %d times; the "
                        "kernel's table holds %d segments per bucket (use a "
                        "smaller bucket cap)" % (len(segs), ADAM_MAX_SEGMENTS))
                ends = [s[0] for s in segs]
                if (ends != sorted(ends) or ends[-1] != bk["p"].numel()
                        or bk["p"].numel() >= 2 ** 31):
                    raise RuntimeError("FusedAdam: malformed decay table")
                dev = bk["p"].device
                bk["seg_end"] = torch.tensor([s[0] for s in segs],
                                             dtype=torch.int32, device=dev)
                bk["seg_wd"] = torch.tensor([s[1] for s in segs],
                                            dtype=torch.float32, device=dev)

    def _materialize(self):
        if self._buckets is not None:
            return self._buckets
        r = self._reducer
        if r is None:
            raise RuntimeError("FusedAdam needs a BucketedAllReducer (call attach())")
        out = []
        for b in r._buckets:
            if b.param_flat is None:
                raise RuntimeError("FusedAdam requires flatten_params=True buckets")
            offsets = []
            off = 0
            for p in b.params:
                offsets.append((off, p.numel()))
                off += p.numel()
            out.append({"p": b.param_flat, "g": b.buffer,
                        "m": torch.zeros_like(b.param_flat),
                        "v": torch.zeros_like(b.param_flat),
                        "params": b.params, "offsets": offsets})
        self._buckets = out
        self._build_tables()
        if out:
            dev = out[0]["p"].device
            if self._step_t is None:
                self._step_t = torch.zeros(1, dtype=torch.int32, device=dev)
            if dev.type == "cuda" and self._lr_dev is None:
                self._lr_dev = torch.full(
                    (1,), self.param_groups[0]["lr"], dtype=torch.float32,
                    device=dev)
        return out

    @torch.no_grad()
    def step(self):
        from .conv import bump_weight_epoch

        bump_weight_epoch()
        buckets = self._materialize()
        if not buckets:
            return
        g0 = self.param_groups[0]
        lr, (b1, b2), eps = g0["lr"], g0["betas"], g0["eps"]
        decoupled = g0["decoupled"]
        self._step_t.add_(1)
        if buckets[0]["p"].is_cuda:
            fused_adam = ext().fused_adam
            for bk in buckets:
                fused_adam(bk["p"], bk["g"], bk["m"], bk["v"], self._step_t,
                           lr, b1, b2, eps, bk["wd"], self.grad_scale,
                           decoupled, self._lr_dev, bk["seg_end"],
                           bk["seg_wd"])
            return
        t = int(self._step_t.item())
        bc1 = 1 - b1 ** t
        bc2 = 1 - b2 ** t
        step_size = lr / bc1
        bc2_sqrt = bc2 ** 0.5
        for bk in buckets:
            p, m, v = bk["p"], bk["m"], bk["v"]
            g = bk["g"]
            if self.grad_scale != 1.0:
                g = g.mul(self.grad_scale)
            start = 0
            for end, wd in bk["segs"]:
                if wd != 0.0:
                    if decoupled:
                        p[start:end].mul_(1 - lr * wd)
                    else:
                        if g is bk["g"]:
                            g = g.clone()
                        g[start:end].add_(p[start:end], alpha=wd)
                start = end
            m.lerp_(g, 1 - b1)
            v.mul_(b2).addcmul_(g, g, value=1 - b2)
            denom = (v.sqrt() / bc2_sqrt).add_(eps)
            p.addcdiv_(m, denom, value=-step_size)

    def zero_grad(self, set_to_none=False):
        if self._reducer is not None:
            self._reducer.zero_grad()

    def state_buffers(self):
        out = []
        for bk in self._materialize():
            out += [bk["m"], bk["v"]]
        if self._step_t is not None:
            out.append(self._step_t)
        return out

    def state_dict(self):
        state = {}
        buckets = self._materialize()
        t = float(self.step_count)
        for bk in buckets:
            for (off, n), p in zip(bk["offsets"], bk["params"]):
                state[self._index[id(p)]] = {
                    "step": torch.tensor(t, dtype=torch.float32),
                    "exp_avg": _view_like(bk["m"][off:off + n], p).clone(),
                    "exp_avg_sq": _view_like(bk["v"][off:off + n], p).clone(),
                }
        state = {k: state[k] for k in sorted(state)}
        groups = [{k: v for k, v in self.param_groups[0].items() if k != "params"}]
        groups[0]["no_decay"] = sorted(self._no_decay)
        groups[0]["params"] = list(range(len(self._all_params)))
        return {"state": state, "param_groups": groups}

    def load_state_dict(self, sd):
        if sd.get("param_groups"):
            src = sd["param_groups"][0]
            if ("decoupled" in src
                    and bool(src["decoupled"]) != self.param_groups[0]["decoupled"]):
                raise ValueError(
                    "FusedAdam: state dict was saved with decoupled=%s, this "
                    "optimizer has decoupled=%s" % (
                        bool(src["decoupled"]),
                        self.param_groups[0]["decoupled"]))
            if ("no_decay" in src
                    and sorted(src["no_decay"]) != sorted(self._no_decay)):
                raise ValueError(
                    "FusedAdam: state dict exempts params %s from weight "
                    "decay, this optimizer %s" % (
                        sorted(src["no_decay"]), sorted(self._no_decay)))
        state = sd.get("state", {})
        steps = []
        for bk in self._materialize():
            for (off, n), p in zip(bk["offsets"], bk["params"]):
                idx = self._index[id(p)]
                ent = state.get(idx, state.get(str(idx)))
                if not ent:
                    continue
                for key, flat in (("exp_avg", bk["m"]), ("exp_avg_sq", bk["v"])):
                    if ent.get(key) is not None:
                        _view_like(flat[off:off + n], p).copy_(
                            ent[key].to(flat.device))
                if ent.get("step") is not None:
                    steps.append(int(float(ent["step"])))
        if steps and self._step_t is not None:
            self._step_t.fill_(max(steps))
        if sd.get("param_groups"):
            src = sd["param_groups"][0]
            g0 = self.param_groups[0]
            for k in ("lr", "eps", "weight_decay"):
                if k in src:
                    g0[k] = float(src[k])
            if "betas" in src:
                g0["betas"] = (float(src["betas"][0]), float(src["betas"][1]))
            if self._lr_dev is not None:
                self._lr_dev.fill_(g0["lr"])
            self._build_tables()


class FusedAdamW(FusedAdam):

    def __init__(self, params, lr=1e-3, betas=(0.9, 0.999), eps=1e-8,
                 weight_decay=1e-2, no_decay=None, grad_scale=1.0,
                 reducer=None, decoupled=True):
        super().__init__(params, lr=lr, betas=betas, eps=eps,
                         weight_decay=weight_decay, decoupled=decoupled,
                         no_decay=no_decay, grad_scale=grad_scale,
                         reducer=reducer)
```

edl_amd/ops/conv.py:

```python
import torch
import torch.nn as nn
import torch.nn.functional as F

import os

from . import available, ext

_CONV1X1 = os.environ.get("EDL_CONV1X1", "hip")

_WGRAD = os.environ.get("EDL_WGRAD", "tn")
_WGRAD3_MAXC = int(os.environ.get("EDL_WGRAD3_TN_MAXC", "128"))


class _Conv1x1Hip(torch.autograd.Function):

    @staticmethod
    def forward(ctx, x2d, w_param, w_bf16, wt_cached, grad_tgt,
                part_out=None):
        ctx.save_for_backward(x2d)
        ctx.wt = wt_cached
        ctx.w_dtype = w_param.dtype
        ctx.grad_tgt = grad_tgt
        if part_out is not None:
            y2d, part = ext().gemm_bt_stats(x2d, w_bf16)
            part_out.append(part)
            return y2d
        return ext().gemm_bt(x2d, w_bf16)

    @staticmethod
    def backward(ctx, dy2d):
        (x2d,) = ctx.saved_tensors
        dy2d = dy2d.contiguous()
        e = ext()
        dx = e.gemm_bt(dy2d, ctx.wt)
        if _WGRAD == "tn":
            if ctx.grad_tgt is not None:
                e.gemm_tn_splitk(
                    dy2d, x2d, 0,
                    ctx.grad_tgt.view(ctx.grad_tgt.shape[0], -1))
                return dx, None, None, None, None, None
            dw = e.gemm_tn_splitk(dy2d, x2d, 0)
        else:
            dw = e.gemm_bt_splitk(e.transpose_pad(dy2d), e.transpose_pad(x2d), 0)
        if dw.dtype != ctx.w_dtype:
            dw = dw.to(ctx.w_dtype)
        return dx, dw, None, None, None, None


_CONV3X3 = os.environ.get("EDL_CONV3X3", "hip")

_GROUPED_MINC = int(os.environ.get("EDL_CONV3X3_GROUPED_MINC", "16"))

_BN_STATS_FUSED = os.environ.get("EDL_BN_STATS_FUSED", "1") == "1"

_PAD_ONCE = os.environ.get("EDL_PAD_ONCE", "1") == "1"
_BN_PAD_OUT = os.environ.get("EDL_BN_PAD_OUT", "1") == "1"
_BN_PAD_DX = os.environ.get("EDL_BN_PAD_DX", "0") == "1"


def padded_interior(xp):
    return xp[:, 1:-1, 1:-1, :].permute(0, 3, 1, 2)


def is_interior_of(t, xp):
    if xp is None or xp.dim() != 4 or t.dim() != 4:
        return False
    n, hp, wp, c = xp.shape
    return (t.dtype == xp.dtype and t.device == xp.device
            and xp.is_contiguous()
            and tuple(t.shape) == (n, c, hp - 2, wp - 2)
            and tuple(t.stride()) == (hp * wp * c, 1, wp * c, c)
            and t.data_ptr() == xp.data_ptr()
            + (wp + 1) * c * xp.element_size())


_weight_epoch = 0


def bump_weight_epoch():
    global _weight_epoch
    _weight_epoch += 1


def _out_hw(h, w, stride):
    return (h - 1) // stride + 1, (w - 1) // stride + 1


def _nchw_view(y2d, n, h, w):
    return y2d.view(n, h, w, y2d.shape[1]).permute(0, 3, 1, 2)


def _repack_w3(weight):
    co, ci = weight.shape[0], weight.shape[1]
    return weight.permute(0, 2, 3, 1).reshape(co, 9 * ci).to(
        torch.bfloat16).contiguous()


class _Conv3x3Hip(torch.autograd.Function):

    @staticmethod
    def forward(ctx, x, w_param, w_bf16, w3_cached, w3rot_cached, stride,
                grad_tgt, part_out=None, xp=None, dyp_holder=None):
        e = ext()
        n, ci, h, w = x.shape
        ctx.padded = xp is not None or _PAD_ONCE
        if ctx.padded:
            if xp is None:
                xp = e.pad_nhwc(x)
            ctx.save_for_backward(xp, w_bf16)
        else:
            ctx.save_for_backward(x, w_bf16)
        ctx.x_shape = (n, ci, h, w)
        ctx.dyp_holder = dyp_holder
        ctx.stride = stride
        ctx.w3rot = w3rot_cached
        ctx.w_dtype = w_param.dtype
        ctx.grad_tgt = grad_tgt
        if part_out is not None:
            if ctx.padded:
                y2d, part = e.conv3x3_fwd_stats_padded(xp, w3_cached, stride,
                                                       h, w)
            else:
                y2d, part = e.conv3x3_fwd_stats(x, w3_cached, stride)
            if part is not None:
                part_out.append(part)
        elif ctx.padded:
            y2d = e.conv3x3_fwd_padded(xp, w3_cached, stride, h, w)
        else:
            y2d = e.conv3x3_fwd(x, w3_cached, stride)
        return _nchw_view(y2d, n, *_out_hw(h, w, stride))

    @staticmethod
    def backward(ctx, dy):
        x, weight = ctx.saved_tensors
        stride = ctx.stride
        n, cin, h, w = ctx.x_shape
        ho, wo = _out_hw(h, w, stride)
        dyp = None
        if ctx.dyp_holder:
            cand = ctx.dyp_holder.pop()
            if is_interior_of(dy, cand):
                dyp = cand
        if dyp is None:
            dy = dy.contiguous(memory_format=torch.channels_last)
        e = ext()
        if dyp is None and stride == 2 and ctx.w3rot is None:
            dx = torch.nn.grad.conv2d_input(
                [n, cin, h, w], weight, dy, stride=(stride, stride),
                padding=(1, 1))
        else:
            if dyp is not None and stride == 1:
                dx2d = e.conv3x3_fwd_padded(dyp, ctx.w3rot, 1, ho, wo)
            elif dyp is not None:
                dx2d = e.conv3x3s2_dgrad_padded(dyp, ctx.w3rot, h, w)
            elif stride == 1:
                dx2d = e.conv3x3_fwd(dy.to(torch.bfloat16), ctx.w3rot, 1)
            else:
                dx2d = e.conv3x3s2_dgrad(dy.to(torch.bfloat16), ctx.w3rot,
                                         h, w)
            dx = _nchw_view(dx2d, n, h, w)
        co = weight.shape[0]
        ci = weight.shape[1]
        none9 = (None,) * 9
        if dyp is not None:
            dya = dyp
        else:
            dya = dy.permute(0, 2, 3, 1).reshape(-1, co).to(torch.bfloat16)
        if dyp is not None or (_WGRAD == "tn" and ci <= _WGRAD3_MAXC):
            if ctx.padded:
                dw3 = e.gemm_tn3x3_splitk_padded(dya, x, h, w, stride, 0,
                                                 ctx.grad_tgt)
            else:
                dw3 = e.gemm_tn3x3_splitk(dya, x, stride, 0, ctx.grad_tgt)
            if ctx.grad_tgt is not None:
                return (dx,) + none9
        else:
            dw3 = e.gemm_bt_splitk(
                e.transpose_pad(dya),
                e.conv3x3_wgrad_operand_padded(x, h, w, stride) if ctx.padded
                else e.conv3x3_wgrad_operand(x, stride), 0)
        dw = dw3.view(co, 3, 3, ci).permute(0, 3, 1, 2)
        if dw.dtype != ctx.w_dtype:
            dw = dw.to(ctx.w_dtype)
        return (dx, dw) + none9[1:]


def _small_cpt(cin):
    if cin <= 16:
        return 16
    if cin <= 32:
        return 32
    return 64


def _repack_w3_small(weight, cpt):
    co, ci = weight.shape[0], weight.shape[1]
    taps_pad = {16: 12, 32: 10, 64: 9}[cpt]
    out = torch.zeros(64, taps_pad, cpt, dtype=torch.bfloat16,
                      device=weight.device)
    out[:co, :9, :ci] = (weight.detach().permute(0, 2, 3, 1)
                         .reshape(co, 9, ci).to(torch.bfloat16))
    return out.reshape(64, taps_pad * cpt).contiguous()


class _Conv3x3SmallHip(torch.autograd.Function):

    @staticmethod
    def forward(ctx, x, w_param, w3s, w3srot, stride, cout, part_out=None):
        ctx.save_for_backward(x)
        ctx.stride = stride
        ctx.w3srot = w3srot
        ctx.w_dtype = w_param.dtype
        ctx.w_shape = tuple(w_param.shape)
        cpt = _small_cpt(x.shape[1])
        if part_out is not None:
            y2d, part = ext().conv3x3_small_fwd_stats(x, w3s, cout, cpt,
                                                      stride)
            part_out.append(part)
        else:
            y2d = ext().conv3x3_small_fwd(x, w3s, cout, cpt, stride)
        n, _, h, w = x.shape
        return _nchw_view(y2d, n, *_out_hw(h, w, stride))

    @staticmethod
    def backward(ctx, dy):
        (x,) = ctx.saved_tensors
        co, ci = ctx.w_shape[0], ctx.w_shape[1]
        dy = dy.contiguous(memory_format=torch.channels_last)
        dyb = dy.to(torch.bfloat16)
        dx = None
        if ctx.needs_input_grad[0] and ctx.w3srot is not None:
            n, _, h, w = x.shape
            cpt = _small_cpt(co)
            dx2d = ext().conv3x3_small_fwd(dyb, ctx.w3srot, ci, cpt, 1)
            dx = _nchw_view(dx2d, n, h, w)
        route = os.environ.get("EDL_STEM_WGRAD", "miopen")
        if route == "tn":
            dy2d = dyb.permute(0, 2, 3, 1).reshape(-1, co)
            if co < 64:
                dy2d = F.pad(dy2d, (0, 64 - co))
            cfull = ext().gemm_tn3x3_small(dy2d.contiguous(), x, ctx.stride)
            cinp = max(8, 1 << max(0, (ci - 1).bit_length()))
            dw = (cfull[:co, :9 * cinp].view(co, 3, 3, cinp)
                  .permute(0, 3, 1, 2)[:, :ci].contiguous())
        elif route == "unfold":
            dy2d = dyb.permute(0, 2, 3, 1).reshape(-1, co)
            xu = F.unfold(x, 3, padding=1, stride=ctx.stride)
            xu2d = xu.permute(0, 2, 1).reshape(-1, ci * 9)
            dw = (dy2d.t() @ xu2d).float().view(co, ci, 3, 3)
        else:
            dw = torch.nn.grad.conv2d_weight(
                x, ctx.w_shape, dyb, stride=(ctx.stride, ctx.stride),
                padding=(1, 1))
        if dw.dtype != ctx.w_dtype:
            dw = dw.to(ctx.w_dtype)
        return dx, dw, None, None, None, None, None


_S2D_TAP_ORDER = [(1, 1), (1, 0), (1, 2), (0, 1), (2, 1),
                  (0, 0), (0, 2), (2, 0), (2, 2)]


def _repack_w3_s2dgrad(weight):
    co, ci = weight.shape[0], weight.shape[1]
    w = weight.detach()
    slabs = torch.stack([w[:, :, dy, dx] for dy, dx in _S2D_TAP_ORDER])
    return (slabs.permute(2, 0, 1).reshape(ci, 9 * co)
            .to(torch.bfloat16).contiguous())


def _repack_w3_grouped(weight):
    co, cpg = weight.shape[0], weight.shape[1]
    if cpg >= 64:
        return _repack_w3(weight.detach())
    w = weight.detach().to(torch.bfloat16)
    gpt = 64 // cpg
    out = torch.zeros(co, 3, 3, 64, dtype=torch.bfloat16, device=w.device)
    pos = (torch.arange(co, device=w.device) // cpg) % gpt
    for p in range(gpt):
        m = pos == p
        out[m, :, :, p * cpg:(p + 1) * cpg] = w[m].permute(0, 2, 3, 1)
    return out.reshape(co, 9 * 64).contiguous()


class Conv2dFast(nn.Conv2d):

    def _direct_grad(self):
        w = self.weight
        if (getattr(w, "_edl_direct_grad", False) and w.grad is not None
                and w.grad.dtype == torch.float32
                and torch.is_grad_enabled() and self.training):
            return w.grad
        return None

    def _cached(self, key, fn):
        epoch = _weight_epoch if self.weight.requires_grad else -1
        cache = getattr(self, "_w_cache", None)
        if cache is None or cache[0] != epoch:
            cache = (epoch, {})
            self._w_cache = cache
        d = cache[1]
        if key not in d:
            d[key] = fn()
        return d[key]

    def prefill_derived(self):
        if not self.weight.requires_grad or not self.weight.is_cuda:
            return
        if not available():
            return
        cache = getattr(self, "_w_cache", None)
        if cache is None or not cache[1]:
            return
        old_keys = list(cache[1].keys())
        co, ci = self.out_channels, self.in_channels
        mb = getattr(self.weight, "_edl_bf16", None)
        cl = getattr(self.weight, "_edl_phys_shape", None) is not None
        builders = {}
        if mb is not None and self.kernel_size == (1, 1):
            builders["wt_t"] = lambda: ext().transpose_pad(mb.view(co, ci))
        if mb is not None and cl and self.kernel_size == (3, 3):
            w3v = mb.permute(0, 2, 3, 1).reshape(co, 9 * ci)
            builders["w3rot"] = lambda: ext().repack_dgrad_w3(w3v, ci, 0)
            builders["w3s2d"] = lambda: ext().repack_dgrad_w3(w3v, ci, 1)
        if self._is_small3x3():
            builders["w3srot"] = self._build_w3srot
        for k in old_keys:
            b = builders.get(k)
            if b is not None:
                self._cached(k, b)

    def pop_bn_part(self):
        p = getattr(self, "_bn_part", None)
        self._bn_part = None
        return p

    def pop_dy_pad(self):
        p = getattr(self, "_dy_pad", None)
        self._dy_pad = None
        return p

    def _is_same3x3(self):
        return (self.kernel_size == (3, 3)
                and self.padding == (1, 1)
                and self.stride[0] == self.stride[1]
                and self.stride[0] in (1, 2)
                and self.bias is None)

    def _is_dense3x3(self):
        return (self._is_same3x3()
                and self.groups == 1
                and self.in_channels % 64 == 0
                and self.out_channels % 64 == 0)

    def _is_small3x3(self):
        return (self._is_same3x3()
                and self.groups == 1
                and self.in_channels <= 64
                and self.out_channels <= 64
                and (self.in_channels % 64 != 0
                     or self.out_channels % 64 != 0))

    def _is_grouped3x3(self):
        cpg = self.in_channels // self.groups
        return (self._is_same3x3()
                and self.groups > 1
                and self.in_channels == self.out_channels
                and cpg >= _GROUPED_MINC
                and cpg in (16, 32, 64, 128)
                and self.in_channels % 64 == 0)

    def takes_padded(self):
        return (_PAD_ONCE and _BN_PAD_OUT and _CONV3X3 == "hip"
                and available() and self._is_dense3x3())

    def _build_w3srot(self):
        return _repack_w3_small(
            self.weight.detach().permute(1, 0, 2, 3).flip(2, 3),
            _small_cpt(self.out_channels))

    def forward(self, x, bn_stats=False, dx_pad=False):
        self._bn_part = None
        self._dy_pad = None
        bn_stats = bn_stats and _BN_STATS_FUSED
        if _CONV3X3 == "hip" and x.is_cuda and available():
            bf16 = x.dtype == torch.bfloat16
            if bf16 and self._is_dense3x3():
                return self._forward_dense3x3(x, bn_stats, dx_pad)
            if ((bf16 or (x.dtype == torch.float32
                          and torch.is_autocast_enabled()))
                    and os.environ.get("EDL_CONV3X3_SMALL", "1") == "1"
                    and self._is_small3x3()):
                return self._forward_small3x3(x, bn_stats)
            if (bf16 and self._is_grouped3x3()
                    and not (torch.is_grad_enabled() and
                             (x.requires_grad or self.weight.requires_grad))):
                return self._forward_grouped3x3(x)
        if (
            _CONV1X1 != "miopen"
            and x.is_cuda
            and self.kernel_size == (1, 1)
            and self.groups == 1
            and self.padding == (0, 0)
            and self.bias is None
        ):
            return self._forward_1x1(x, bn_stats)
        return super().forward(x)

    def _forward_dense3x3(self, x, bn_stats, dx_pad):
        xp = getattr(x, "_edl_xp", None) if _PAD_ONCE else None
        if not is_interior_of(x, xp):
            xp = None
            if not x.is_contiguous(memory_format=torch.channels_last):
                x = x.contiguous(memory_format=torch.channels_last)
        co, ci = self.out_channels, self.in_channels
        cl = getattr(self.weight, "_edl_phys_shape", None) is not None
        mb = getattr(self.weight, "_edl_bf16", None)
        if mb is not None:
            w_bf16 = mb
            wsrc = mb
        else:
            w_bf16 = self._cached("w_bf16", lambda: self.weight.detach().to(
                torch.bfloat16).contiguous())
            wsrc = self.weight.detach()
        if cl and mb is not None:
            w3 = mb.permute(0, 2, 3, 1).reshape(co, 9 * ci)
        else:
            w3 = self._cached("w3", lambda: _repack_w3(wsrc))
        if cl and mb is not None:
            mode = 0 if self.stride[0] == 1 else 1
            w3rot = self._cached(
                "w3rot" if mode == 0 else "w3s2d",
                lambda: ext().repack_dgrad_w3(w3, ci, mode))
        elif self.stride[0] == 1:
            w3rot = self._cached("w3rot", lambda: _repack_w3(
                wsrc.permute(1, 0, 2, 3).flip(2, 3)))
        else:
            w3rot = self._cached("w3s2d", lambda: _repack_w3_s2dgrad(wsrc))
        gather_wgrad = _WGRAD == "tn" and ci <= _WGRAD3_MAXC
        grad_tgt = None
        if cl and ci <= _WGRAD3_MAXC:
            grad_tgt = self._direct_grad()
            if grad_tgt is not None:
                grad_tgt = grad_tgt.permute(0, 2, 3, 1).reshape(co, 9 * ci)
        holder = [] if bn_stats else None
        dyp_holder = None
        if (dx_pad and _PAD_ONCE and _BN_PAD_DX and gather_wgrad
                and w3rot is not None and torch.is_grad_enabled()):
            dyp_holder = []
        y = _Conv3x3Hip.apply(x, self.weight, w_bf16, w3, w3rot,
                              self.stride[0], grad_tgt, holder, xp,
                              dyp_holder)
        if holder:
            self._bn_part = holder[0]
        self._dy_pad = dyp_holder
        return y

    def _forward_small3x3(self, x, bn_stats):
        if x.dtype != torch.bfloat16:
            x = x.to(torch.bfloat16)
        if not x.is_contiguous(memory_format=torch.channels_last):
            x = x.contiguous(memory_format=torch.channels_last)
        cpt = _small_cpt(self.in_channels)
        w3s = self._cached("w3s", lambda: _repack_w3_small(
            self.weight.detach(), cpt))
        w3srot = None
        if self.stride[0] == 1 and x.requires_grad:
            w3srot = self._cached("w3srot", self._build_w3srot)
        holder = [] if bn_stats else None
        y = _Conv3x3SmallHip.apply(x, self.weight, w3s, w3srot,
                                   self.stride[0], self.out_channels, holder)
        if holder:
            self._bn_part = holder[0]
        return y

    def _forward_grouped3x3(self, x):
        if not x.is_contiguous(memory_format=torch.channels_last):
            x = x.contiguous(memory_format=torch.channels_last)
        w3g = self._cached("w3g", lambda: _repack_w3_grouped(self.weight))
        y2d = ext().conv3x3_grouped_fwd(x, w3g, self.stride[0])
        n, _, h, w = x.shape
        return _nchw_view(y2d, n, *_out_hw(h, w, self.stride[0]))

    def _forward_1x1(self, x, bn_stats):
        n, c, h, w = x.shape
        sh, sw = self.stride
        if sh != 1 or sw != 1:
            x = x[:, :, ::sh, ::sw].contiguous(memory_format=torch.channels_last)
            n, c, h, w = x.shape
        if not x.is_contiguous(memory_format=torch.channels_last):
            x = x.contiguous(memory_format=torch.channels_last)
        co = self.out_channels
        x2d = x.permute(0, 2, 3, 1).reshape(n * h * w, c)
        wt = self.weight.view(co, c)
        if not (_CONV1X1 == "hip" and available()
                and x2d.dtype == torch.bfloat16
                and c % 64 == 0 and co % 64 == 0):
            return _nchw_view(x2d @ wt.t(), n, h, w)
        mb = getattr(self.weight, "_edl_bf16", None)
        if mb is not None:
            w_bf16 = mb.view(co, c)
            wt_t = self._cached("wt_t", lambda: ext().transpose_pad(
                mb.view(co, c)))
        else:
            w_bf16 = self._cached("w_bf16", lambda: self.weight.detach()
                                  .view(co, c).to(torch.bfloat16).contiguous())
            wt_t = self._cached("wt_t", lambda: self.weight.detach().view(
                co, c).to(torch.bfloat16).t().contiguous())
        grad_tgt = self._direct_grad()
        if grad_tgt is not None and not grad_tgt.is_contiguous():
            grad_tgt = None
        holder = [] if bn_stats else None
        y2d = _Conv1x1Hip.apply(x2d, wt, w_bf16, wt_t, grad_tgt, holder)
        if holder:
            self._bn_part = holder[0]
        return _nchw_view(y2d, n, h, w)
```

edl_amd/ops/sgd.py:

```python
import torch

from . import available, ext
from ..train.bucketed_ddp import _view_like


class FusedSGD:
    handles_grad_scale = True

    def __init__(self, params, lr=0.1, momentum=0.9, weight_decay=1e-4, grad_scale=1.0,
                 reducer=None):
        self.defaults = dict(lr=lr, momentum=momentum, weight_decay=weight_decay)
        self.param_groups = [dict(self.defaults, params=[p for p in params if p.requires_grad])]
        self.grad_scale = grad_scale
        self._reducer = reducer
        self._buckets = None
        self._use_ext = available() and torch.cuda.is_available()
        self._lr_dev = None
        if reducer is not None:
            self.attach(reducer)

    def attach(self, reducer):
        self._reducer = reducer
        self._buckets = None
        reducer._attached_opt = self
        return self

    def set_lr(self, lr):
        for g in self.param_groups:
            g["lr"] = float(lr)
        if self._lr_dev is not None:
            self._lr_dev.fill_(float(lr))

    def _materialize(self):
        if self._buckets is not None:
            return self._buckets
        r = self._reducer
        if r is None:
            raise RuntimeError("FusedSGD needs a BucketedAllReducer (call attach())")
        out = []
        for b in r._buckets:
            if b.param_flat is None:
                raise RuntimeError("FusedSGD requires flatten_params=True buckets")
            m = torch.zeros_like(b.param_flat)
            offsets = []
            off = 0
            for p in b.params:
                offsets.append((off, p.numel()))
                off += p.numel()
            out.append({"p": b.param_flat, "g": b.buffer, "m": m,
                        "params": b.params, "offsets": offsets})
        self._buckets = out
        if self._use_ext and out and out[0]["p"].is_cuda and self._lr_dev is None:
            self._lr_dev = torch.full(
                (1,), self.param_groups[0]["lr"], dtype=torch.float32,
                device=out[0]["p"].device)
        return out

    @torch.no_grad()
    def step(self, momentum=None, weight_decay=None):
        from .conv import bump_weight_epoch

        bump_weight_epoch()
        g0 = self.param_groups[0]
        lr, mu, wd = g0["lr"], g0["momentum"], g0["weight_decay"]
        if momentum is not None:
            mu = float(momentum)
        if weight_decay is not None:
            wd = float(weight_decay)
        for bk in self._materialize():
            if self._use_ext and bk["p"].is_cuda:
                ext().fused_sgd(bk["p"], bk["g"], bk["m"], lr, mu, wd,
                                self.grad_scale, self._lr_dev)
            else:
                g = bk["g"]
                if self.grad_scale != 1.0:
                    g = g.mul(self.grad_scale)
                g = g.add(bk["p"], alpha=wd)
                bk["m"].mul_(mu).add_(g)
                bk["p"].add_(bk["m"], alpha=-lr)

    def zero_grad(self, set_to_none=False):
        if self._reducer is not None:
            self._reducer.zero_grad()

    def state_dict(self):
        state = {}
        idx = 0
        for bk in self._materialize():
            for (off, n), p in zip(bk["offsets"], bk["params"]):
                state[idx] = {"momentum_buffer": _view_like(bk["m"][off:off + n], p).clone()}
                idx += 1
        groups = [{k: v for k, v in self.param_groups[0].items() if k != "params"}]
        groups[0]["params"] = list(range(idx))
        return {"state": state, "param_groups": groups}

    def load_state_dict(self, sd):
        state = sd.get("state", {})
        idx = 0
        for bk in self._materialize():
            for (off, n), p in zip(bk["offsets"], bk["params"]):
                ent = state.get(idx, state.get(str(idx)))
                if ent is not None and "momentum_buffer" in ent and ent["momentum_buffer"] is not None:
                    _view_like(bk["m"][off:off + n], p).copy_(
                        ent["momentum_buffer"].to(bk["m"].device)
                    )
                idx += 1
        if sd.get("param_groups"):
            for k in ("lr", "momentum", "weight_decay"):
                if k in sd["param_groups"][0]:
                    self.param_groups[0][k] = sd["param_groups"][0][k]
            if self._lr_dev is not None:
                self._lr_dev.fill_(float(self.param_groups[0]["lr"]))
```

edl_amd/train/engine.py:

```python
import os
import time

import torch
import torch.nn.functional as F

from ..models import build_model
from ..utils.log import get_logger
from . import dist as edist
from .bucketed_ddp import BucketedAllReducer
from .checkpoint import CheckpointManager

log = get_logger("edl.engine")

_MARKERS = os.environ.get("EDL_PROFILE_MARKERS") == "1"


class _mark:
    __slots__ = ("name",)

    def __init__(self, name):
        self.name = name

    def __enter__(self):
        if _MARKERS:
            torch.cuda.nvtx.range_push(self.name)

    def __exit__(self, *exc):
        if _MARKERS:
            torch.cuda.nvtx.range_pop()


def piecewise_lr(base_lr, epoch, boundaries=(30, 60, 90), decay=0.1, warmup_epochs=5,
                 step_in_epoch=0.0):
    e = epoch + step_in_epoch
    if e < warmup_epochs:
        return base_lr * (e + 1e-9) / warmup_epochs
    mult = 1.0
    for b in boundaries:
        if epoch >= b:
            mult *= decay
    return base_lr * mult


class DynamicLossScaler:

    def __init__(self, init_scale=2.0 ** 15, growth_factor=2.0,
                 backoff_factor=0.5, growth_interval=2000):
        self.value = float(init_scale)
        self.growth_factor = growth_factor
        self.backoff_factor = backoff_factor
        self.growth_interval = growth_interval
        self._good_steps = 0

    def update(self, found_inf):
        if found_inf:
            self.value = max(1.0, self.value * self.backoff_factor)
            self._good_steps = 0
            return False
        self._good_steps += 1
        if self._good_steps >= self.growth_interval:
            self.value *= self.growth_factor
            self._good_steps = 0
        return True


class TrainerEngine:
    def __init__(
        self,
        model="resnet50_vd",
        per_device_batch=32,
        num_classes=1000,
        base_lr=0.1,
        momentum=0.9,
        weight_decay=1e-4,
        label_smoothing=0.1,
        dtype="bf16",
        channels_last=True,
        bucket_mb=25,
        checkpoint_dir=None,
        use_hip_ops=True,
        graph_capture=None,
        kd_teacher=None,
        kd_alpha=1.0,
        recompute=False,
        dgc=False,
        dgc_ratio=0.01,
        dgc_rampup=0,
        dgc_momentum_correction=False,
        dgc_sparsity=None,
        dgc_rampup_step=1,
        fused_ce=False,
        track_accuracy=False,
        optimizer="momentum",
        betas=(0.9, 0.999),
        eps=1e-8,
        no_decay_1d=False,
    ):
        self.model_name = model
        self.per_device_batch = per_device_batch
        self.num_classes = num_classes
        self.base_lr = base_lr
        self.momentum = momentum
        self.weight_decay = weight_decay
        self.label_smoothing = label_smoothing
        self.dtype = {"bf16": torch.bfloat16, "fp16": torch.float16,
                      "fp32": torch.float32}[dtype]
        self.scaler = DynamicLossScaler() if self.dtype == torch.float16 else None
        self.channels_last = channels_last
        self.bucket_mb = bucket_mb
        self.checkpoint_dir = checkpoint_dir
        self.use_hip_ops = use_hip_ops
        self.graph_capture = graph_capture
        self.kd_teacher = kd_teacher
        self.kd_alpha = kd_alpha
        self.recompute = recompute
        self.dgc_cfg = (dgc, dgc_ratio, dgc_rampup)
        self.dgc = None
        self.dgc_momentum_correction = bool(dgc_momentum_correction)
        self.dgc_sparsity = (tuple(dgc_sparsity) if dgc_sparsity
                             else (1.0 - dgc_ratio,))
        self.dgc_rampup_step = dgc_rampup_step
        if dgc and self.dgc_momentum_correction and self.scaler is not None:
            raise ValueError(
                "DGC momentum correction cannot run under the fp16 loss "
                "scaler: a changing loss scale corrupts the accumulated "
                "gradients (use bf16 or fp32)")
        if optimizer not in ("momentum", "adam", "adamw"):
            raise ValueError("optimizer must be momentum, adam or adamw")
        if optimizer != "momentum" and dgc:
            raise ValueError("DGC needs the momentum optimizer, not %s"
                             % optimizer)
        self.optimizer = optimizer
        self.betas = (float(betas[0]), float(betas[1]))
        self.eps = float(eps)
        self.no_decay_1d = bool(no_decay_1d)
        self.fused_ce = fused_ce
        self.track_accuracy = track_accuracy
        self.last_rank = None

        self.env = None
        self.device = None
        self.model = None
        self.reducer = None
        self.opt = None
        self.ckpt = None
        self.start_epoch = 0
        self.start_step = 0
        self.global_step = 0
        self._graph = None
        self._static = {}
        self._prefill_stream = None
        self._prefill_mods = None

    def setup(self, env=None):
        self.env, self.device = edist.init_from_env(env)
        torch.manual_seed(42 + self.env.global_rank)
        self.model = build_model(self.model_name, num_classes=self.num_classes)
        self.model.to(self.device)
        if (self.device.type == "cuda"
                and os.environ.get("EDL_PREFILL_DERIVED", "0") == "1"):
            self._prefill_stream = torch.cuda.Stream()
        if self.channels_last and self.device.type == "cuda":
            self.model.to(memory_format=torch.channels_last)
        if self.use_hip_ops and self.device.type == "cuda":
            from .. import ops

            ops.assert_hip_ops_available(self.model)
            self._mark_channels_last_conv_weights()
        if self.recompute and hasattr(self.model, "stages"):
            import torch.utils.checkpoint as ckpt_mod

            class _Recompute(torch.nn.Module):
                def __init__(self, inner):
                    super().__init__()
                    self.inner = inner

                def forward(self, x):
                    if self.training and torch.is_grad_enabled():
                        return ckpt_mod.checkpoint(self.inner, x, use_reentrant=False)
                    return self.inner(x)

            self.model.stages = torch.nn.Sequential(
                *[_Recompute(s) for s in self.model.stages]
            )

        self.reducer = BucketedAllReducer(
            self.model.parameters(), bucket_cap_mb=self.bucket_mb
        )
        if self.dgc_cfg[0] and not self.dgc_momentum_correction:
            from .dgc import DGCCompressor

            self.dgc = DGCCompressor(self.reducer, self.dgc_cfg[1],
                                     self.dgc_cfg[2])
        self.opt = self._build_optimizer()
        if self.dgc_cfg[0] and self.dgc_momentum_correction:
            from .dgc import DGCMomentum

            self.dgc = DGCMomentum(
                self.reducer, self.opt, self.momentum, self.weight_decay,
                rampup_begin_step=self.dgc_cfg[2],
                rampup_step=self.dgc_rampup_step, sparsity=self.dgc_sparsity)
        if self.checkpoint_dir:
            self.ckpt = CheckpointManager(self.checkpoint_dir)
            self._resume()
        self.reducer.broadcast_params(src=0)
        self._broadcast_opt_state(src=0)
        from ..ops.conv import bump_weight_epoch

        bump_weight_epoch()
        self._init_bf16_mirrors()
        self.reducer.register_rebuild_callback(self._init_bf16_mirrors)
        edist.barrier(self.device)
        return self

    def _mark_channels_last_conv_weights(self):
        from ..ops.conv import Conv2dFast

        for m in self.model.modules():
            if (isinstance(m, Conv2dFast) and m.kernel_size == (3, 3)
                    and m.groups == 1 and m.bias is None
                    and m.in_channels % 64 == 0 and m.out_channels % 64 == 0
                    and m.padding == (1, 1)):
                w = m.weight
                w._edl_phys_shape = (w.shape[0], 3, 3, w.shape[1])
                w._edl_phys_perm = (0, 3, 1, 2)

    def _broadcast_opt_state(self, src=0):
        import torch.distributed as dist

        if not (dist.is_initialized() and dist.get_world_size() > 1):
            return
        if hasattr(self.opt, "state_buffers"):
            for t in self.opt.state_buffers():
                dist.broadcast(t, src=src)
        elif hasattr(self.opt, "_materialize"):
            for bk in self.opt._materialize():
                dist.broadcast(bk["m"], src=src)

    def _init_bf16_mirrors(self):
        self._bf16_mirrors = []
        if not (self.use_hip_ops and self.device.type == "cuda"):
            return
        for b in self.reducer._buckets:
            if b.param_flat is None or b.param_flat.dtype != torch.float32:
                continue
            mirror = torch.empty_like(b.param_flat, dtype=torch.bfloat16)
            self._bf16_mirrors.append((mirror, b.param_flat))
            off = 0
            from .bucketed_ddp import _view_like
            for p in b.params:
                p._edl_bf16 = _view_like(mirror[off:off + p.numel()], p)
                off += p.numel()
        self._refresh_bf16_mirrors()

    def _refresh_bf16_mirrors(self):
        for mirror, flat in getattr(self, "_bf16_mirrors", ()):
            mirror.copy_(flat, non_blocking=True)

    def _build_optimizer(self):
        if self.optimizer != "momentum":
            from ..ops.adam import FusedAdam

            return FusedAdam(
                self.model.parameters(), lr=self.base_lr, betas=self.betas,
                eps=self.eps, weight_decay=self.weight_decay,
                decoupled=self.optimizer == "adamw",
                no_decay=(lambda p: p.ndim <= 1) if self.no_decay_1d else None,
                grad_scale=self.reducer.grad_scale, reducer=self.reducer,
            )
        from ..ops.sgd import FusedSGD

        return FusedSGD(
            self.model.parameters(), lr=self.base_lr, momentum=self.momentum,
            weight_decay=self.weight_decay, grad_scale=self.reducer.grad_scale,
            reducer=self.reducer,
        )

    @property
    def world_size(self):
        return edist.world_size()

    @property
    def global_batch(self):
        return self.per_device_batch * self.world_size

    def scaled_lr(self, epoch, step_in_epoch=0.0):
        if self.optimizer != "momentum":
            return self.base_lr
        lr = self.base_lr * self.global_batch / 256.0
        return piecewise_lr(lr, epoch, step_in_epoch=step_in_epoch)

    def set_lr(self, lr):
        if hasattr(self.opt, "set_lr"):
            self.opt.set_lr(lr)
        else:
            for g in self.opt.param_groups:
                g["lr"] = lr

    def _resume(self):
        got = self.ckpt.load(map_location="cpu")
        if got is None:
            if self.env.is_rank0:
                log.info("no checkpoint in %s; fresh start", self.checkpoint_dir)
            return
        model_state, opt_state, ts = got
        self.model.load_state_dict(model_state)
        if opt_state is not None:
            try:
                self.opt.load_state_dict(opt_state)
            except (ValueError, KeyError) as e:
                log.warning("optimizer state mismatch (%s); reset", e)
        if ts.get("mid_epoch"):
            self.start_epoch = int(ts.get("epoch_no", 0))
            self.start_step = int(ts.get("step_in_epoch", 0))
        else:
            self.start_epoch = int(ts.get("epoch_no", -1)) + 1
            self.start_step = 0
        self.global_step = int(ts.get("global_step", 0))
        if self.env.is_rank0:
            log.info(
                "resumed from checkpoint v%s: epoch %d step %d, global_step %d (world=%d)",
                ts.get("_version"), self.start_epoch, self.start_step,
                self.global_step, self.world_size,
            )

    def save_checkpoint(self, epoch, extra=None, blocking=False):
        if self.ckpt is None or not self.env.is_rank0:
            return None
        ts = {"epoch_no": epoch, "global_step": self.global_step,
              "world_size": self.world_size, "total_batch_size": self.global_batch}
        ts.update(extra or {})
        return self.ckpt.save(
            self.model.state_dict(), ts, optimizer_state=self.opt.state_dict(),
            blocking=blocking,
        )

    def _hard_loss(self, logits, labels, labels_b=None, lam=None):
        if not (self.fused_ce or self.track_accuracy or labels_b is not None):
            return F.cross_entropy(logits.float(), labels,
                                   label_smoothing=self.label_smoothing)
        from ..ops.functional import softmax_cross_entropy

        loss, rank = softmax_cross_entropy(
            logits, labels, label_smoothing=self.label_smoothing,
            labels_b=labels_b, lam=lam, return_rank=True)
        if self.track_accuracy and labels_b is None:
            self.last_rank = rank
        return loss

    def _loss(self, logits, labels, teacher_logits=None, labels_b=None,
              lam=None):
        if teacher_logits is not None:
            from ..ops.functional import kd_soft_cross_entropy

            kd = kd_soft_cross_entropy(logits, teacher_logits)
            if self.kd_alpha >= 1.0:
                return kd
            ce = self._hard_loss(logits, labels, labels_b, lam)
            return self.kd_alpha * kd + (1 - self.kd_alpha) * ce
        return self._hard_loss(logits, labels, labels_b, lam)

    def train_step(self, images, labels, teacher_logits=None, labels_b=None,
                   lam=None):
        self.reducer.zero_grad()
        self._prefill_derived_async()
        with _mark("edl.forward"):
            with torch.autocast(device_type=self.device.type, dtype=self.dtype,
                                enabled=self.dtype != torch.float32):
                logits = self.model(images)
            loss = self._loss(logits, labels, teacher_logits, labels_b, lam)
        with _mark("edl.backward"):
            if self._prefill_stream is not None:
                torch.cuda.current_stream().wait_stream(self._prefill_stream)
            if self.scaler is not None:
                (loss * self.scaler.value).backward()
            else:
                loss.backward()
        with _mark("edl.allreduce_finalize"):
            opt_kw = {}
            if self.dgc_momentum_correction and self.dgc is not None:
                self.dgc.step(global_step=self.global_step + 1)
                opt_kw = self.dgc.opt_overrides()
            elif self.dgc is not None:
                self.dgc.step()
            else:
                self.reducer.finalize()
        with _mark("edl.optimizer"):
            inv_scale = 1.0
            if self.scaler is not None:
                flags = torch.stack(
                    [torch.isfinite(b.buffer).all()
                     for b in self.reducer._buckets])
                found_inf = not bool(flags.all().item())
                if not self.scaler.update(found_inf):
                    self.global_step += 1
                    return loss
                inv_scale = 1.0 / self.scaler.value
            if getattr(self.opt, "handles_grad_scale", False):
                if inv_scale != 1.0:
                    base = self.opt.grad_scale
                    self.opt.grad_scale = base * inv_scale
                    try:
                        self.opt.step(**opt_kw)
                    finally:
                        self.opt.grad_scale = base
                else:
                    self.opt.step(**opt_kw)
            else:
                scale = self.reducer.grad_scale * inv_scale
                if scale != 1.0:
                    for b in self.reducer._buckets:
                        b.buffer.mul_(scale)
                self.opt.step()
            self._refresh_bf16_mirrors()
        self.global_step += 1
        return loss

    def _prefill_derived_async(self):
        if self._prefill_stream is None:
            return
        mods = self._prefill_mods
        if mods is None:
            from ..ops.conv import Conv2dFast

            mods = [m for m in self.model.modules()
                    if isinstance(m, Conv2dFast)]
            self._prefill_mods = mods
        cur = torch.cuda.current_stream()
        self._prefill_stream.wait_stream(cur)
        with torch.cuda.stream(self._prefill_stream):
            for m in mods:
                m.prefill_derived()

    def maybe_capture(self, images, labels, labels_b=None, lam=None):
        if self.device.type != "cuda" or self._graph is not None:
            return False
        if self.scaler is not None:
            return False
        if self.dgc_momentum_correction and self.dgc is not None:
            return False
        want = self.graph_capture
        if want is None:
            env = os.environ.get("EDL_GRAPH_CAPTURE")
            if env is not None:
                want = env == "1"
            else:
                want = self.world_size == 1
        if not want:
            return False
        try:
            self._static["x"] = images.clone()
            self._static["y"] = labels.clone()
            mix = {}
            if labels_b is not None:
                self._static["y_b"] = labels_b.clone()
                self._static["lam"] = lam.to(torch.float32).clone()
                mix = {"labels_b": self._static["y_b"],
                       "lam": self._static["lam"]}
            torch.cuda.synchronize()
            s = torch.cuda.Stream()
            s.wait_stream(torch.cuda.current_stream())
            with torch.cuda.stream(s):
                for _ in range(3):
                    self.train_step(self._static["x"], self._static["y"],
                                    **mix)
            torch.cuda.current_stream().wait_stream(s)
            torch.cuda.synchronize()
            g = torch.cuda.CUDAGraph()
            step_before = self.global_step
            with torch.cuda.graph(g):
                self._static["loss"] = self.train_step(
                    self._static["x"], self._static["y"], **mix)
            self.global_step = step_before
            self._graph = g
            log.info("captured train step as hipGraph")
            return True
        except Exception as e:
            log.warning("hipGraph capture failed (%s); running eager", e)
            self._graph = None
            self._static = {}
            return False

    def replay_step(self, images, labels, labels_b=None, lam=None):
        if self._graph is not None:
            if (labels_b is not None) != ("y_b" in self._static):
                raise ValueError(
                    "replay_step: the captured step was %s mixup labels"
                    % ("built with" if "y_b" in self._static else
                       "built without"))
            self._static["x"].copy_(images, non_blocking=True)
            self._static["y"].copy_(labels, non_blocking=True)
            if labels_b is not None:
                self._static["y_b"].copy_(labels_b, non_blocking=True)
                self._static["lam"].copy_(lam, non_blocking=True)
            self._graph.replay()
            self.global_step += 1
            return self._static["loss"]
        return self.train_step(images, labels, labels_b=labels_b, lam=lam)

    def evaluate(self, loader, steps):
        from ..ops.bnrelu import BNReLU2d
        from ..ops.conv import bump_weight_epoch
        from ..ops.functional import softmax_cross_entropy

        bump_weight_epoch()
        for m in self.model.modules():
            if isinstance(m, BNReLU2d):
                m._eval_ver = None
        self._refresh_bf16_mirrors()

        was_training = self.model.training
        self.model.eval()
        acc = torch.zeros(4, dtype=torch.float64, device=self.device)
        seen = 0
        try:
            with torch.no_grad():
                for _ in range(steps):
                    x, y = loader.next()
                    with torch.autocast(device_type=self.device.type,
                                        dtype=self.dtype,
                                        enabled=self.dtype != torch.float32):
                        logits = self.model(x)
                    loss, rank = softmax_cross_entropy(
                        logits, y, label_smoothing=0.0, return_rank=True)
                    n = y.shape[0]
                    seen += n
                    acc[:3] += torch.stack([
                        loss.double() * n, (rank < 1).sum().double(),
                        (rank < 5).sum().double()])
        finally:
            self.model.train(was_training)
        acc[3] = seen
        import torch.distributed as dist

        if dist.is_initialized() and dist.get_world_size() > 1:
            if dist.get_backend() != "nccl":
                acc = acc.cpu()
            dist.all_reduce(acc, op=dist.ReduceOp.SUM)
        loss_sum, c1, c5, count = acc.tolist()
        div = max(count, 1.0)
        return {"loss": loss_sum / div, "acc1": c1 / div, "acc5": c5 / div,
                "samples": int(count)}

    def train_epoch(self, epoch, loader, steps, log_every=50, on_step=None,
                    start_step=0):
        self.model.train()
        t0 = time.monotonic()
        imgs_done = 0
        loss = None
        for it in range(start_step, steps):
            self.set_lr(self.scaled_lr(epoch, it / max(1, steps)))
            loss = self.replay_step(*loader.next())
            imgs_done += self.global_batch
            if on_step:
                on_step(epoch, it)
            if log_every and (it + 1) % log_every == 0 and self.env.is_rank0:
                if self.device.type == "cuda":
                    torch.cuda.synchronize()
                dt = time.monotonic() - t0
                log.info(
                    "epoch %d step %d/%d loss=%.4f %.1f img/s (world=%d)",
                    epoch, it + 1, steps, loss.item(), imgs_done / dt, self.world_size,
                )
        if self.device.type == "cuda":
            torch.cuda.synchronize()
        dt = time.monotonic() - t0
        return {"epoch": epoch, "steps": steps, "time_s": dt,
                "img_per_s": imgs_done / dt,
                "loss": float(loss.item()) if loss is not None else None}
```

Measured before the change: 3836 img/s.

## Fuse bf16 mirror write into optimizer and batch conv weight repacks

The fused SGD and Adam kernels gain variants that write the bf16 parameter mirror directly. This removes the separate fp32-to-bf16 copy pass after each step. A new batched repack kernel and arena also build all derived conv weight layouts (transposed, rotated, space-to-depth, small) in one launch after the mirror refresh, replacing per-conv derivation or prefill. This adds a table-driven repack path and more code complexity, and depends on alignment checks.

```diff
diff --git a/edl_amd/csrc/common.h b/edl_amd/csrc/common.h
--- a/edl_amd/csrc/common.h
+++ b/edl_amd/csrc/common.h
@@ -28,3 +28,14 @@
   for (int off = 32; off > 0; off >>= 1) v = fmaxf(v, __shfl_down(v, off, 64));
   return v;
 }
+
+__device__ __forceinline__ void store_bf16x4(__hip_bfloat16* dst,
+                                             const float4 v) {
+  ulong1 packed;
+  __hip_bfloat16* pv = reinterpret_cast<__hip_bfloat16*>(&packed);
+  pv[0] = __float2bfloat16(v.x);
+  pv[1] = __float2bfloat16(v.y);
+  pv[2] = __float2bfloat16(v.z);
+  pv[3] = __float2bfloat16(v.w);
+  *reinterpret_cast<ulong1*>(__builtin_assume_aligned(dst, 8)) = packed;
+}
diff --git a/edl_amd/csrc/fused_adam.hip b/edl_amd/csrc/fused_adam.hip
--- a/edl_amd/csrc/fused_adam.hip
+++ b/edl_amd/csrc/fused_adam.hip
@@ -40,88 +40,35 @@
 
 }
 
-extern "C" __global__ void fused_adam_f32(
-    float* __restrict__ p, const float* __restrict__ g, float* __restrict__ m,
-    float* __restrict__ v, const int* __restrict__ step_dev,
-    const float* __restrict__ lr_dev, const float lr_host, const float b1,
-    const float b2, const float omb1, const float omb2, const float ln_b1,
-    const float ln_b2, const float eps, const float wd, const float scale,
-    const int decoupled, const long long n, const int* __restrict__ seg_end,
-    const float* __restrict__ seg_wd, const int nseg) {
-  extern __shared__ int s_tab[];
-  int* s_end = s_tab;
-  float* s_wd = reinterpret_cast<float*>(s_tab + nseg);
-  if (nseg > 0) {
-    for (int k = threadIdx.x; k < nseg; k += blockDim.x) {
-      s_end[k] = seg_end[k];
-      s_wd[k] = seg_wd[k];
-    }
-    __syncthreads();
-  }
+#define FUSED_ADAM_KERNEL fused_adam_f32
+#define FUSED_ADAM_MIRROR 0
+#include "fused_adam_body.h"
+#undef FUSED_ADAM_KERNEL
+#undef FUSED_ADAM_MIRROR
 
-  AdamCoef c;
-  c.lr = lr_dev ? *lr_dev : lr_host;
-  const int t = *step_dev;
-  const float tf = (float)(t > 1 ? t : 1);
-  c.b1 = b1; c.b2 = b2; c.omb1 = omb1; c.omb2 = omb2;
-  c.eps = eps; c.scale = scale; c.decoupled = decoupled != 0;
-  c.step_size = c.lr / -expm1f(tf * ln_b1);
-  c.sqrt_bc2 = sqrtf(-expm1f(tf * ln_b2));
-
-  const long long n4 = n >> 2;
-  const float4* g4 = reinterpret_cast<const float4*>(g);
-  float4* p4 = reinterpret_cast<float4*>(p);
-  float4* m4 = reinterpret_cast<float4*>(m);
-  float4* v4 = reinterpret_cast<float4*>(v);
-  long long i = (long long)blockIdx.x * blockDim.x + threadIdx.x;
-  const long long stride = (long long)gridDim.x * blockDim.x;
-  int s = 0;
-  for (; i < n4; i += stride) {
-    float4 pg = g4[i], pp = p4[i], pm = m4[i], pv = v4[i];
-    float w0 = wd, w1 = wd, w2 = wd, w3 = wd;
-    if (nseg > 0) {
-      const int e = (int)(i << 2);
-      s = adam_find_seg(s_end, s, nseg, e);
-      int q = s;
-      w0 = s_wd[q];
-      q = adam_next_seg(s_end, q, nseg, e + 1);
-      w1 = s_wd[q];
-      q = adam_next_seg(s_end, q, nseg, e + 2);
-      w2 = s_wd[q];
-      q = adam_next_seg(s_end, q, nseg, e + 3);
-      w3 = s_wd[q];
-    }
-    adam_elem(c, w0, pg.x, pp.x, pm.x, pv.x);
-    adam_elem(c, w1, pg.y, pp.y, pm.y, pv.y);
-    adam_elem(c, w2, pg.z, pp.z, pm.z, pv.z);
-    adam_elem(c, w3, pg.w, pp.w, pm.w, pv.w);
-    m4[i] = pm;
-    v4[i] = pv;
-    p4[i] = pp;
-  }
-  for (long long j = (n4 << 2) + (long long)blockIdx.x * blockDim.x + threadIdx.x;
-       j < n; j += stride) {
-    float w = wd;
-    if (nseg > 0) w = s_wd[adam_find_seg(s_end, 0, nseg, (int)j)];
-    float pj = p[j], mj = m[j], vj = v[j];
-    adam_elem(c, w, g[j], pj, mj, vj);
-    m[j] = mj;
-    v[j] = vj;
-    p[j] = pj;
-  }
-}
+#define FUSED_ADAM_KERNEL fused_adam_f32_mirror
+#define FUSED_ADAM_MIRROR 1
+#include "fused_adam_body.h"
+#undef FUSED_ADAM_KERNEL
+#undef FUSED_ADAM_MIRROR
 
 extern "C" void launch_fused_adam_f32(
     float* p, const float* g, float* m, float* v, const int* step_dev,
     const float* lr_dev, float lr, float b1, float b2, float omb1, float omb2,
     float ln_b1, float ln_b2, float eps, float wd, float scale, int decoupled,
     long long n, const int* seg_end, const float* seg_wd, int nseg,
-    hipStream_t stream) {
+    void* mirror, hipStream_t stream) {
   const int block = 256;
   const int grid = elementwise_grid((n + 3) / 4, block);
   const size_t lds = (size_t)nseg * (sizeof(int) + sizeof(float));
-  hipLaunchKernelGGL(fused_adam_f32, dim3(grid), dim3(block), lds, stream, p,
-                     g, m, v, step_dev, lr_dev, lr, b1, b2, omb1, omb2, ln_b1,
-                     ln_b2, eps, wd, scale, decoupled, n, seg_end, seg_wd,
-                     nseg);
+  if (mirror)
+    hipLaunchKernelGGL(fused_adam_f32_mirror, dim3(grid), dim3(block), lds,
+                       stream, p, g, m, v, step_dev, lr_dev, lr, b1, b2, omb1,
+                       omb2, ln_b1, ln_b2, eps, wd, scale, decoupled, n,
+                       seg_end, seg_wd, nseg, (__hip_bfloat16*)mirror);
+  else
+    hipLaunchKernelGGL(fused_adam_f32, dim3(grid), dim3(block), lds, stream,
+                       p, g, m, v, step_dev, lr_dev, lr, b1, b2, omb1, omb2,
+                       ln_b1, ln_b2, eps, wd, scale, decoupled, n, seg_end,
+                       seg_wd, nseg);
 }
diff --git a/edl_amd/csrc/fused_adam_body.h b/edl_amd/csrc/fused_adam_body.h
--- /dev/null
+++ b/edl_amd/csrc/fused_adam_body.h
@@ -0,0 +1,80 @@
+extern "C" __global__ void FUSED_ADAM_KERNEL(
+    float* __restrict__ p, const float* __restrict__ g, float* __restrict__ m,
+    float* __restrict__ v, const int* __restrict__ step_dev,
+    const float* __restrict__ lr_dev, const float lr_host, const float b1,
+    const float b2, const float omb1, const float omb2, const float ln_b1,
+    const float ln_b2, const float eps, const float wd, const float scale,
+    const int decoupled, const long long n, const int* __restrict__ seg_end,
+    const float* __restrict__ seg_wd, const int nseg
+#if FUSED_ADAM_MIRROR
+    , __hip_bfloat16* __restrict__ mirror
+#endif
+) {
+  extern __shared__ int s_tab[];
+  int* s_end = s_tab;
+  float* s_wd = reinterpret_cast<float*>(s_tab + nseg);
+  if (nseg > 0) {
+    for (int k = threadIdx.x; k < nseg; k += blockDim.x) {
+      s_end[k] = seg_end[k];
+      s_wd[k] = seg_wd[k];
+    }
+    __syncthreads();
+  }
+
+  AdamCoef c;
+  c.lr = lr_dev ? *lr_dev : lr_host;
+  const int t = *step_dev;
+  const float tf = (float)(t > 1 ? t : 1);
+  c.b1 = b1; c.b2 = b2; c.omb1 = omb1; c.omb2 = omb2;
+  c.eps = eps; c.scale = scale; c.decoupled = decoupled != 0;
+  c.step_size = c.lr / -expm1f(tf * ln_b1);
+  c.sqrt_bc2 = sqrtf(-expm1f(tf * ln_b2));
+
+  const long long n4 = n >> 2;
+  const float4* g4 = reinterpret_cast<const float4*>(g);
+  float4* p4 = reinterpret_cast<float4*>(p);
+  float4* m4 = reinterpret_cast<float4*>(m);
+  float4* v4 = reinterpret_cast<float4*>(v);
+  long long i = (long long)blockIdx.x * blockDim.x + threadIdx.x;
+  const long long stride = (long long)gridDim.x * blockDim.x;
+  int s = 0;
+  for (; i < n4; i += stride) {
+    float4 pg = g4[i], pp = p4[i], pm = m4[i], pv = v4[i];
+    float w0 = wd, w1 = wd, w2 = wd, w3 = wd;
+    if (nseg > 0) {
+      const int e = (int)(i << 2);
+      s = adam_find_seg(s_end, s, nseg, e);
+      int q = s;
+      w0 = s_wd[q];
+      q = adam_next_seg(s_end, q, nseg, e + 1);
+      w1 = s_wd[q];
+      q = adam_next_seg(s_end, q, nseg, e + 2);
+      w2 = s_wd[q];
+      q = adam_next_seg(s_end, q, nseg, e + 3);
+      w3 = s_wd[q];
+    }
+    adam_elem(c, w0, pg.x, pp.x, pm.x, pv.x);
+    adam_elem(c, w1, pg.y, pp.y, pm.y, pv.y);
+    adam_elem(c, w2, pg.z, pp.z, pm.z, pv.z);
+    adam_elem(c, w3, pg.w, pp.w, pm.w, pv.w);
+    m4[i] = pm;
+    v4[i] = pv;
+    p4[i] = pp;
+#if FUSED_ADAM_MIRROR
+    store_bf16x4(mirror + (i << 2), pp);
+#endif
+  }
+  for (long long j = (n4 << 2) + (long long)blockIdx.x * blockDim.x + threadIdx.x;
+       j < n; j += stride) {
+    float w = wd;
+    if (nseg > 0) w = s_wd[adam_find_seg(s_end, 0, nseg, (int)j)];
+    float pj = p[j], mj = m[j], vj = v[j];
+    adam_elem(c, w, g[j], pj, mj, vj);
+    m[j] = mj;
+    v[j] = vj;
+    p[j] = pj;
+#if FUSED_ADAM_MIRROR
+    mirror[j] = __float2bfloat16(pj);
+#endif
+  }
+}
diff --git a/edl_amd/csrc/fused_sgd.hip b/edl_amd/csrc/fused_sgd.hip
--- a/edl_amd/csrc/fused_sgd.hip
+++ b/edl_amd/csrc/fused_sgd.hip
@@ -1,49 +1,29 @@
 #include "common.h"
 #include "launchers.h"
 
-extern "C" __global__ void fused_sgd_f32(
-    float* __restrict__ p, const float* __restrict__ g, float* __restrict__ m,
-    const float lr_host, const float mu, const float wd, const float scale,
-    const long long n, const float* __restrict__ lr_dev) {
-  const float lr = lr_dev ? *lr_dev : lr_host;
-  const long long n4 = n >> 2;
-  const float4* g4 = reinterpret_cast<const float4*>(g);
-  float4* p4 = reinterpret_cast<float4*>(p);
-  float4* m4 = reinterpret_cast<float4*>(m);
-  long long i = (long long)blockIdx.x * blockDim.x + threadIdx.x;
-  const long long stride = (long long)gridDim.x * blockDim.x;
-  for (; i < n4; i += stride) {
-    float4 pg = g4[i], pp = p4[i], pm = m4[i];
-    float d0 = fmaf(scale, pg.x, wd * pp.x);
-    float d1 = fmaf(scale, pg.y, wd * pp.y);
-    float d2 = fmaf(scale, pg.z, wd * pp.z);
-    float d3 = fmaf(scale, pg.w, wd * pp.w);
-    pm.x = fmaf(mu, pm.x, d0);
-    pm.y = fmaf(mu, pm.y, d1);
-    pm.z = fmaf(mu, pm.z, d2);
-    pm.w = fmaf(mu, pm.w, d3);
-    pp.x = fmaf(-lr, pm.x, pp.x);
-    pp.y = fmaf(-lr, pm.y, pp.y);
-    pp.z = fmaf(-lr, pm.z, pp.z);
-    pp.w = fmaf(-lr, pm.w, pp.w);
-    m4[i] = pm;
-    p4[i] = pp;
-  }
-  for (long long j = (n4 << 2) + (long long)blockIdx.x * blockDim.x + threadIdx.x;
-       j < n; j += stride) {
-    float d = fmaf(scale, g[j], wd * p[j]);
-    float mv = fmaf(mu, m[j], d);
-    m[j] = mv;
-    p[j] = fmaf(-lr, mv, p[j]);
-  }
-}
+#define FUSED_SGD_KERNEL fused_sgd_f32
+#define FUSED_SGD_MIRROR 0
+#include "fused_sgd_body.h"
+#undef FUSED_SGD_KERNEL
+#undef FUSED_SGD_MIRROR
+
+#define FUSED_SGD_KERNEL fused_sgd_f32_mirror
+#define FUSED_SGD_MIRROR 1
+#include "fused_sgd_body.h"
+#undef FUSED_SGD_KERNEL
+#undef FUSED_SGD_MIRROR
 
 extern "C" void launch_fused_sgd_f32(float* p, const float* g, float* m,
                                      float lr, float mu, float wd, float scale,
                                      long long n, const float* lr_dev,
-                                     hipStream_t stream) {
+                                     void* mirror, hipStream_t stream) {
   const int block = 256;
   const int grid = elementwise_grid((n + 3) / 4, block);
-  hipLaunchKernelGGL(fused_sgd_f32, dim3(grid), dim3(block), 0, stream,
-                     p, g, m, lr, mu, wd, scale, n, lr_dev);
+  if (mirror)
+    hipLaunchKernelGGL(fused_sgd_f32_mirror, dim3(grid), dim3(block), 0,
+                       stream, p, g, m, lr, mu, wd, scale, n, lr_dev,
+                       (__hip_bfloat16*)mirror);
+  else
+    hipLaunchKernelGGL(fused_sgd_f32, dim3(grid), dim3(block), 0, stream,
+                       p, g, m, lr, mu, wd, scale, n, lr_dev);
 }
diff --git a/edl_amd/csrc/fused_sgd_body.h b/edl_amd/csrc/fused_sgd_body.h
--- /dev/null
+++ b/edl_amd/csrc/fused_sgd_body.h
@@ -0,0 +1,49 @@
+extern "C" __global__ void FUSED_SGD_KERNEL(
+    float* __restrict__ p, const float* __restrict__ g, float* __restrict__ m,
+    const float lr_host, const float mu, const float wd, const float scale,
+    const long long n, const float* __restrict__ lr_dev
+#if FUSED_SGD_MIRROR
+    , __hip_bfloat16* __restrict__ mirror
+#endif
+) {
+  const float lr = lr_dev ? *lr_dev : lr_host;
+  const long long n4 = n >> 2;
+  const float4* g4 = reinterpret_cast<const float4*>(g);
+  float4* p4 = reinterpret_cast<float4*>(p);
+  float4* m4 = reinterpret_cast<float4*>(m);
+  long long i = (long long)blockIdx.x * blockDim.x + threadIdx.x;
+  const long long stride = (long long)gridDim.x * blockDim.x;
+  for (; i < n4; i += stride) {
+    float4 pg = g4[i], pp = p4[i], pm = m4[i];
+    float d0 = fmaf(scale, pg.x, wd * pp.x);
+    float d1 = fmaf(scale, pg.y, wd * pp.y);
+    float d2 = fmaf(scale, pg.z, wd * pp.z);
+    float d3 = fmaf(scale, pg.w, wd * pp.w);
+    pm.x = fmaf(mu, pm.x, d0);
+    pm.y = fmaf(mu, pm.y, d1);
+    pm.z = fmaf(mu, pm.z, d2);
+    pm.w = fmaf(mu, pm.w, d3);
+    pp.x = fmaf(-lr, pm.x, pp.x);
+    pp.y = fmaf(-lr, pm.y, pp.y);
+    pp.z = fmaf(-lr, pm.z, pp.z);
+    pp.w = fmaf(-lr, pm.w, pp.w);
+    m4[i] = pm;
+    p4[i] = pp;
+#if FUSED_SGD_MIRROR
+    store_bf16x4(mirror + (i << 2), pp);
+#endif
+  }
+  for (long long j = (n4 << 2) + (long long)blockIdx.x * blockDim.x + threadIdx.x;
+       j < n; j += stride) {
+    float d = fmaf(scale, g[j], wd * p[j]);
+    float mv = fmaf(mu, m[j], d);
+    m[j] = mv;
+#if FUSED_SGD_MIRROR
+    const float pj = fmaf(-lr, mv, p[j]);
+    p[j] = pj;
+    mirror[j] = __float2bfloat16(pj);
+#else
+    p[j] = fmaf(-lr, mv, p[j]);
+#endif
+  }
+}
diff --git a/edl_amd/csrc/launchers.h b/edl_amd/csrc/launchers.h
--- a/edl_amd/csrc/launchers.h
+++ b/edl_amd/csrc/launchers.h
@@ -7,7 +7,8 @@
 
 void launch_fused_sgd_f32(float* p, const float* g, float* m, float lr,
                           float mu, float wd, float scale, long long n,
-                          const float* lr_dev, hipStream_t stream);
+                          const float* lr_dev, void* mirror,
+                          hipStream_t stream);
 
 constexpr int kAdamMaxSegments = 1024;
 void launch_fused_adam_f32(float* p, const float* g, float* m, float* v,
@@ -16,7 +17,7 @@
                            float ln_b1, float ln_b2, float eps, float wd,
                            float scale, int decoupled, long long n,
                            const int* seg_end, const float* seg_wd, int nseg,
-                           hipStream_t stream);
+                           void* mirror, hipStream_t stream);
 
 void launch_kd_ce_fwd_f32(const float* s, const float* t, float* lpr, int B,
                           int C, hipStream_t stream);
@@ -130,6 +131,17 @@
 void launch_repack_dgrad_w3(const void* in, void* out, int Co, int Ci,
                             int mode, hipStream_t s);
 void launch_cast_bf16_zero(float* src, void* dst, long long n, hipStream_t s);
+constexpr int kRepackJobWords = 8;
+constexpr int kRepackMaxJobs = 1024;
+constexpr int kRepackMaxSources = 16;
+constexpr int kRepackSmallElems = 2048;
+enum RepackKind {
+  kRepackT = 0, kRepackRot = 1, kRepackS2d = 2, kRepackSmall = 3,
+  kRepackSmallRot = 4
+};
+void launch_repack_weights_batched(const int* table, int njobs, int ntiles,
+                                   const void* const* sources, int nsources,
+                                   void* arena, hipStream_t s);
 
 void launch_maxpool3x3s2_fwd(const void* x, void* y, unsigned char* idx,
                              int N, int H, int W, int Ho, int Wo, int C,
diff --git a/edl_amd/csrc/module.cpp b/edl_amd/csrc/module.cpp
--- a/edl_amd/csrc/module.cpp
+++ b/edl_amd/csrc/module.cpp
@@ -187,9 +187,24 @@
                          cur_stream());
 }
 
+void* opt_mirror_ptr(const c10::optional<torch::Tensor>& mirror,
+                     const torch::Tensor& p, const char* who) {
+  if (!mirror.has_value()) return nullptr;
+  TORCH_CHECK(mirror->is_cuda() && mirror->device() == p.device() &&
+                  mirror->scalar_type() == torch::kBFloat16 &&
+                  mirror->is_contiguous(),
+              who, ": mirror must be a contiguous bf16 tensor on p's GPU");
+  TORCH_CHECK(mirror->numel() == p.numel(), who,
+              ": mirror and p differ in length");
+  TORCH_CHECK(reinterpret_cast<uintptr_t>(mirror->data_ptr()) % 8 == 0, who,
+              ": mirror must be 8-byte aligned (4 bf16 per store)");
+  return mirror->data_ptr();
+}
+
 void fused_sgd(torch::Tensor p, torch::Tensor g, torch::Tensor m, double lr,
                double momentum, double weight_decay, double grad_scale,
-               c10::optional<torch::Tensor> lr_dev) {
+               c10::optional<torch::Tensor> lr_dev,
+               c10::optional<torch::Tensor> mirror) {
   TORCH_CHECK(p.is_cuda() && g.is_cuda() && m.is_cuda(), "fused_sgd: GPU tensors required");
   TORCH_CHECK(p.scalar_type() == torch::kFloat32 && g.scalar_type() == torch::kFloat32 &&
                   m.scalar_type() == torch::kFloat32,
@@ -204,9 +219,11 @@
                 "fused_sgd: lr_dev must be a fp32 GPU scalar");
     lrp = lr_dev->data_ptr<float>();
   }
+  void* mirp = opt_mirror_ptr(mirror, p, "fused_sgd");
   launch_fused_sgd_f32(p.data_ptr<float>(), g.data_ptr<float>(), m.data_ptr<float>(),
                        (float)lr, (float)momentum, (float)weight_decay,
-                       (float)grad_scale, (long long)p.numel(), lrp, cur_stream());
+                       (float)grad_scale, (long long)p.numel(), lrp, mirp,
+                       cur_stream());
 }
 
 
@@ -253,7 +270,8 @@
                 double grad_scale, bool decoupled,
                 c10::optional<torch::Tensor> lr_dev,
                 c10::optional<torch::Tensor> seg_end,
-                c10::optional<torch::Tensor> seg_wd) {
+                c10::optional<torch::Tensor> seg_wd,
+                c10::optional<torch::Tensor> mirror) {
   TORCH_CHECK(p.is_cuda() && g.is_cuda() && m.is_cuda() && v.is_cuda(),
               "fused_adam: GPU tensors required");
   TORCH_CHECK(p.scalar_type() == torch::kFloat32 &&
@@ -314,6 +332,7 @@
     wdp = seg_wd->data_ptr<float>();
     nseg = (int)seg_end->numel();
   }
+  void* mirp = opt_mirror_ptr(mirror, p, "fused_adam");
   if (n == 0) return;
   launch_fused_adam_f32(
       p.data_ptr<float>(), g.data_ptr<float>(), m.data_ptr<float>(),
@@ -321,7 +340,7 @@
       (float)beta1, (float)beta2, (float)(1.0 - beta1), (float)(1.0 - beta2),
       (float)std::log(beta1), (float)std::log(beta2), (float)eps,
       (float)weight_decay, (float)grad_scale, decoupled ? 1 : 0, n, endp, wdp,
-      nseg, cur_stream());
+      nseg, mirp, cur_stream());
 }
 
 torch::Tensor kd_ce_forward(torch::Tensor s, torch::Tensor t) {
@@ -795,6 +814,95 @@
   return out;
 }
 
+struct RepackExtent {
+  long long src, dst;
+  int tiles;
+};
+
+RepackExtent repack_job_extent(int kind, long long co, long long ci, int cpt) {
+  if (kind == kRepackT || kind == kRepackRot || kind == kRepackS2d) {
+    TORCH_CHECK(co >= 64 && ci >= 64 && co % 64 == 0 && ci % 64 == 0 &&
+                    co * ci * 9 < (1LL << 31),
+                "repack_weights_batched: tile kinds need Co, Ci % 64 == 0");
+    const long long taps = kind == kRepackT ? 1 : 9;
+    return {taps * co * ci, taps * co * ci,
+            (int)(taps * (co / 64) * (ci / 64))};
+  }
+  TORCH_CHECK(kind == kRepackSmall || kind == kRepackSmallRot,
+              "repack_weights_batched: unknown job kind ", kind);
+  TORCH_CHECK(cpt == 16 || cpt == 32 || cpt == 64,
+              "repack_weights_batched: cpt must be 16, 32 or 64");
+  const long long rows = kind == kRepackSmall ? co : ci;
+  const long long cols = kind == kRepackSmall ? ci : co;
+  TORCH_CHECK(rows >= 1 && rows <= 64 && cols >= 1 && cols <= cpt,
+              "repack_weights_batched: small kinds need rows <= 64 and "
+              "cols <= cpt");
+  const long long taps_pad = cpt == 16 ? 12 : (cpt == 32 ? 10 : 9);
+  const long long out = 64 * taps_pad * cpt;
+  return {co * ci * 9, out,
+          (int)((out + kRepackSmallElems - 1) / kRepackSmallElems)};
+}
+
+void repack_weights_batched(torch::Tensor table, torch::Tensor table_host,
+                            torch::Tensor arena,
+                            std::vector<torch::Tensor> sources) {
+  TORCH_CHECK(arena.is_cuda() && arena.scalar_type() == torch::kBFloat16 &&
+                  arena.is_contiguous() &&
+                  reinterpret_cast<uintptr_t>(arena.data_ptr()) % 16 == 0,
+              "repack_weights_batched: arena must be contiguous bf16 on the "
+              "GPU, 16-byte aligned");
+  TORCH_CHECK(table.is_cuda() && table.device() == arena.device() &&
+                  table.scalar_type() == torch::kInt32 &&
+                  table.is_contiguous() && table.dim() == 2 &&
+                  table.size(1) == kRepackJobWords,
+              "repack_weights_batched: table must be int32 [njobs, ",
+              kRepackJobWords, "] on the arena's GPU");
+  TORCH_CHECK(!table_host.is_cuda() &&
+                  table_host.scalar_type() == torch::kInt32 &&
+                  table_host.is_contiguous() &&
+                  table_host.sizes() == table.sizes(),
+              "repack_weights_batched: table_host must be the table's host "
+              "copy");
+  const int njobs = (int)table.size(0);
+  TORCH_CHECK(njobs >= 1 && njobs <= kRepackMaxJobs,
+              "repack_weights_batched: 1 <= jobs <= ", kRepackMaxJobs);
+  const int nsrc = (int)sources.size();
+  TORCH_CHECK(nsrc >= 1 && nsrc <= kRepackMaxSources,
+              "repack_weights_batched: 1 <= sources <= ", kRepackMaxSources);
+  const void* srcp[kRepackMaxSources];
+  for (int k = 0; k < nsrc; ++k) {
+    const torch::Tensor& t = sources[k];
+    TORCH_CHECK(t.is_cuda() && t.device() == arena.device() &&
+                    t.scalar_type() == torch::kBFloat16 && t.is_contiguous(),
+                "repack_weights_batched: sources must be contiguous bf16 on "
+                "the arena's GPU");
+    srcp[k] = t.data_ptr();
+  }
+  const int* row = table_host.data_ptr<int>();
+  int tiles = 0;
+  for (int j = 0; j < njobs; ++j, row += kRepackJobWords) {
+    const int kind = row[0], si = row[1];
+    const long long soff = row[2], doff = row[3];
+    const RepackExtent e = repack_job_extent(kind, row[4], row[5], row[7]);
+    TORCH_CHECK(si >= 0 && si < nsrc, "repack_weights_batched: job ", j,
+                " names source ", si);
+    TORCH_CHECK(soff >= 0 && soff + e.src <= sources[si].numel(),
+                "repack_weights_batched: job ", j, " reads outside its source");
+    TORCH_CHECK(doff >= 0 && doff + e.dst <= arena.numel(),
+                "repack_weights_batched: job ", j, " writes outside the arena");
+    const bool tile_kind = kind != kRepackSmall && kind != kRepackSmallRot;
+    TORCH_CHECK(doff % 8 == 0 &&
+                    (!tile_kind ||
+                     (reinterpret_cast<uintptr_t>(srcp[si]) + 2 * soff) % 16 == 0),
+                "repack_weights_batched: job ", j, " is not 16-byte aligned");
+    tiles += e.tiles;
+    TORCH_CHECK(row[6] == tiles, "repack_weights_batched: job ", j,
+                " has cumulative tile end ", row[6], ", expected ", tiles);
+  }
+  launch_repack_weights_batched(table.data_ptr<int>(), njobs, tiles, srcp,
+                                nsrc, arena.data_ptr(), cur_stream());
+}
+
 std::vector<torch::Tensor> maxpool3x3s2_fwd(torch::Tensor x) {
   check_nhwc_bf16(x, "maxpool3x3s2", 8);
   const int N = (int)x.size(0), C = (int)x.size(1);
@@ -1083,7 +1191,7 @@
         "fused flat momentum-SGD update (p,g,m flat fp32; folds grad_scale)",
         py::arg("p"), py::arg("g"), py::arg("m"), py::arg("lr"),
         py::arg("momentum"), py::arg("weight_decay"), py::arg("grad_scale"),
-        py::arg("lr_dev") = py::none());
+        py::arg("lr_dev") = py::none(), py::arg("mirror") = py::none());
   m.def("fused_adam", &fused_adam,
         "fused flat Adam/AdamW update (p,g,m,v flat fp32; step count and lr "
         "read from device scalars; optional per-segment decay table of at "
@@ -1093,7 +1201,7 @@
         py::arg("beta2"), py::arg("eps"), py::arg("weight_decay"),
         py::arg("grad_scale"), py::arg("decoupled"),
         py::arg("lr_dev") = py::none(), py::arg("seg_end") = py::none(),
-        py::arg("seg_wd") = py::none());
+        py::arg("seg_wd") = py::none(), py::arg("mirror") = py::none());
   m.attr("ADAM_MAX_SEGMENTS") = kAdamMaxSegments;
   m.def("dgc_workspace_words", &dgc_workspace_words,
         "int32 words of the (zero-initialised) DGC select workspace");
@@ -1190,6 +1298,16 @@
         "small-channel 3x3 conv (deep stem) -> y2d [M, cout_real]");
   m.def("conv3x3_small_fwd_stats", &conv3x3_small_fwd_stats,
         "stem conv + BN stats partials -> (y2d, part)");
+  m.def("repack_weights_batched", &repack_weights_batched,
+        "rebuild every weight-derived bf16 layout of the job table in ONE "
+        "launch: table int32 [njobs, 8] {kind, source, source offset, "
+        "destination offset, Co, Ci, cumulative tile end, cpt} on the GPU and "
+        "its host copy, arena, sources (the bf16 bucket mirrors)",
+        py::arg("table"), py::arg("table_host"), py::arg("arena"),
+        py::arg("sources"));
+  m.attr("REPACK_MAX_JOBS") = kRepackMaxJobs;
+  m.attr("REPACK_MAX_SOURCES") = kRepackMaxSources;
+  m.attr("REPACK_SMALL_ELEMS") = kRepackSmallElems;
   m.def("repack_dgrad_w3", &repack_dgrad_w3,
         "dgrad weight repack [Co,9Ci]->[Ci,9Co] (mode 0 rot / 1 s2 order)");
   m.def("maxpool3x3s2_fwd", &maxpool3x3s2_fwd,
diff --git a/edl_amd/csrc/transpose.hip b/edl_amd/csrc/transpose.hip
--- a/edl_amd/csrc/transpose.hip
+++ b/edl_amd/csrc/transpose.hip
@@ -3,12 +3,10 @@
 
 using bf16 = __hip_bfloat16;
 
-extern "C" __global__ void transpose_pad_kernel(
+__device__ __forceinline__ void transpose_tile_64(
     const bf16* __restrict__ in, bf16* __restrict__ out, const int M,
-    const int C, const int Mp) {
+    const int C, const int Mp, const int tm0, const int tc0) {
   __shared__ bf16 tile[64][64 + 4];
-  const int tm0 = blockIdx.x * 64;
-  const int tc0 = blockIdx.y * 64;
   const int lr = threadIdx.x >> 3;
   const int lc = (threadIdx.x & 7) * 8;
   for (int half = 0; half < 2; ++half) {
@@ -33,6 +31,12 @@
       *reinterpret_cast<uint4*>(__builtin_assume_aligned(dst, 16)) = *reinterpret_cast<const uint4*>(v);
     }
   }
+}
+
+extern "C" __global__ void transpose_pad_kernel(
+    const bf16* __restrict__ in, bf16* __restrict__ out, const int M,
+    const int C, const int Mp) {
+  transpose_tile_64(in, out, M, C, Mp, blockIdx.x * 64, blockIdx.y * 64);
 }
 
 extern "C" void launch_transpose_pad(const void* in, void* out, int M, int C,
@@ -91,15 +95,11 @@
 
 __constant__ int S2D_ORDER[9] = {4, 3, 5, 1, 7, 0, 2, 6, 8};
 
-extern "C" __global__ void repack_dgrad_w3_kernel(
+__device__ __forceinline__ void repack_w3_tile_64(
     const __hip_bfloat16* __restrict__ in, __hip_bfloat16* __restrict__ out,
-    const int Co, const int Ci, const int mode) {
+    const int Co, const int Ci, const int tap, const int s, const int ci0,
+    const int co0) {
   __shared__ __hip_bfloat16 tile[64][64 + 8];
-  const int s = blockIdx.y;
-  const int tap = mode == 0 ? 8 - s : S2D_ORDER[s];
-  const int tiles_co = Co >> 6;
-  const int ci0 = (blockIdx.x / tiles_co) << 6;
-  const int co0 = (blockIdx.x % tiles_co) << 6;
   const int lane = threadIdx.x & 63;
   const int quad = threadIdx.x >> 6;
   {
@@ -131,12 +131,110 @@
   }
 }
 
+extern "C" __global__ void repack_dgrad_w3_kernel(
+    const __hip_bfloat16* __restrict__ in, __hip_bfloat16* __restrict__ out,
+    const int Co, const int Ci, const int mode) {
+  const int s = blockIdx.y;
+  const int tap = mode == 0 ? 8 - s : S2D_ORDER[s];
+  const int tiles_co = Co >> 6;
+  const int ci0 = (blockIdx.x / tiles_co) << 6;
+  const int co0 = (blockIdx.x % tiles_co) << 6;
+  repack_w3_tile_64(in, out, Co, Ci, tap, s, ci0, co0);
+}
+
 extern "C" void launch_repack_dgrad_w3(const void* in, void* out, int Co,
                                        int Ci, int mode, hipStream_t s) {
   const dim3 grid((Ci >> 6) * (Co >> 6), 9);
   hipLaunchKernelGGL(repack_dgrad_w3_kernel, grid, dim3(256), 0, s,
                      (const __hip_bfloat16*)in, (__hip_bfloat16*)out, Co, Ci,
                      mode);
+}
+
+struct RepackSources {
+  const __hip_bfloat16* p[kRepackMaxSources];
+};
+
+__device__ __forceinline__ int repack_small_taps_pad(const int cpt) {
+  return cpt == 16 ? 12 : (cpt == 32 ? 10 : 9);
+}
+
+__device__ __forceinline__ void repack_small_chunk(
+    const __hip_bfloat16* __restrict__ in, __hip_bfloat16* __restrict__ out,
+    const int Co, const int Ci, const int cpt, const bool rot, const int t) {
+  const int taps_pad = repack_small_taps_pad(cpt);
+  const int e0 = t * kRepackSmallElems + threadIdx.x * 8;
+  if (e0 >= 64 * taps_pad * cpt) return;
+  const int c0 = e0 % cpt;
+  const int tp = (e0 / cpt) % taps_pad;
+  const int r = e0 / (cpt * taps_pad);
+  const int rows = rot ? Ci : Co, cols = rot ? Co : Ci;
+  const unsigned short* raw = reinterpret_cast<const unsigned short*>(in);
+  unsigned int w[4] = {0u, 0u, 0u, 0u};
+  if (r < rows && tp < 9) {
+#pragma unroll
+    for (int k = 0; k < 8; ++k) {
+      const int c = c0 + k;
+      unsigned int h = 0u;
+      if (c < cols)
+        h = rot ? raw[((long long)c * Ci + r) * 9 + (8 - tp)]
+                : raw[((long long)r * Ci + c) * 9 + tp];
+      w[k >> 1] |= h << ((k & 1) * 16);
+    }
+  }
+  const uint4 v = {w[0], w[1], w[2], w[3]};
+  *reinterpret_cast<uint4*>(__builtin_assume_aligned(out + e0, 16)) = v;
+}
+
+extern "C" __global__ void repack_weights_batched_kernel(
+    const int* __restrict__ table, const int njobs, const RepackSources srcs,
+    __hip_bfloat16* __restrict__ arena) {
+  __shared__ int s_end[kRepackMaxJobs];
+  if (njobs < 1 || njobs > kRepackMaxJobs) return;
+  for (int k = threadIdx.x; k < njobs; k += blockDim.x)
+    s_end[k] = table[k * kRepackJobWords + 6];
+  __syncthreads();
+  const int b = blockIdx.x;
+  int lo = 0, hi = njobs - 1;
+  while (lo < hi) {
+    const int mid = (lo + hi) >> 1;
+    if (s_end[mid] > b) hi = mid; else lo = mid + 1;
+  }
+  const int j = __builtin_amdgcn_readfirstlane(lo);
+  const int* row = table + (long long)j * kRepackJobWords;
+  const int kind = row[0];
+  const int si = min(max(row[1], 0), kRepackMaxSources - 1);
+  const __hip_bfloat16* in = srcs.p[si] + row[2];
+  __hip_bfloat16* out = arena + row[3];
+  const int Co = row[4], Ci = row[5], cpt = row[7];
+  const int t = b - (j > 0 ? s_end[j - 1] : 0);
+  if (t < 0) return;
+  const int tiles_co = Co >> 6, tiles_ci = Ci >> 6;
+  if (kind == kRepackT) {
+    if (t >= tiles_co * tiles_ci) return;
+    transpose_tile_64(in, out, Co, Ci, Co, (t % tiles_co) << 6,
+                      (t / tiles_co) << 6);
+  } else if (kind == kRepackRot || kind == kRepackS2d) {
+    const int per_tap = tiles_co * tiles_ci;
+    if (t >= 9 * per_tap) return;
+    const int s = t / per_tap, xy = t % per_tap;
+    const int tap = kind == kRepackRot ? 8 - s : S2D_ORDER[s];
+    repack_w3_tile_64(in, out, Co, Ci, tap, s, (xy / tiles_co) << 6,
+                      (xy % tiles_co) << 6);
+  } else if (kind == kRepackSmall || kind == kRepackSmallRot) {
+    repack_small_chunk(in, out, Co, Ci, cpt, kind == kRepackSmallRot, t);
+  }
+}
+
+extern "C" void launch_repack_weights_batched(const int* table, int njobs,
+                                              int ntiles,
+                                              const void* const* sources,
+                                              int nsources, void* arena,
+                                              hipStream_t s) {
+  RepackSources srcs;
+  for (int k = 0; k < kRepackMaxSources; ++k)
+    srcs.p[k] = (const __hip_bfloat16*)sources[k < nsources ? k : 0];
+  hipLaunchKernelGGL(repack_weights_batched_kernel, dim3(ntiles), dim3(256),
+                     0, s, table, njobs, srcs, (__hip_bfloat16*)arena);
 }
 
 extern "C" __global__ void cast_bf16_zero_kernel(
diff --git a/edl_amd/ops/adam.py b/edl_amd/ops/adam.py
--- a/edl_amd/ops/adam.py
+++ b/edl_amd/ops/adam.py
@@ -38,14 +38,24 @@
         self._buckets = None
         self._step_t = None
         self._lr_dev = None
+        self._mirrors = {}
+        self._mirrors_written = set()
         if reducer is not None:
             self.attach(reducer)
 
     def attach(self, reducer):
         self._reducer = reducer
         self._buckets = None
+        self._mirrors = {}
         reducer._attached_opt = self
         return self
+
+    def attach_mirrors(self, pairs):
+        self._mirrors = {flat.data_ptr(): mirror for mirror, flat in pairs}
+
+    def pop_mirrors_written(self):
+        out, self._mirrors_written = self._mirrors_written, set()
+        return out
 
     def set_lr(self, lr):
         for g in self.param_groups:
@@ -125,6 +135,7 @@
         from .conv import bump_weight_epoch
 
         bump_weight_epoch()
+        self._mirrors_written = set()
         buckets = self._materialize()
         if not buckets:
             return
@@ -135,10 +146,13 @@
         if buckets[0]["p"].is_cuda:
             fused_adam = ext().fused_adam
             for bk in buckets:
+                mirror = self._mirrors.get(bk["p"].data_ptr())
                 fused_adam(bk["p"], bk["g"], bk["m"], bk["v"], self._step_t,
                            lr, b1, b2, eps, bk["wd"], self.grad_scale,
                            decoupled, self._lr_dev, bk["seg_end"],
-                           bk["seg_wd"])
+                           bk["seg_wd"], mirror)
+                if mirror is not None:
+                    self._mirrors_written.add(bk["p"].data_ptr())
             return
         t = int(self._step_t.item())
         bc1 = 1 - b1 ** t
diff --git a/edl_amd/ops/conv.py b/edl_amd/ops/conv.py
--- a/edl_amd/ops/conv.py
+++ b/edl_amd/ops/conv.py
@@ -5,6 +5,7 @@
 import os
 
 from . import available, ext
+from .weight_repack import small_cpt as _small_cpt
 
 _CONV1X1 = os.environ.get("EDL_CONV1X1", "hip")
 
@@ -183,14 +184,6 @@
         if dw.dtype != ctx.w_dtype:
             dw = dw.to(ctx.w_dtype)
         return (dx, dw) + none9[1:]
-
-
-def _small_cpt(cin):
-    if cin <= 16:
-        return 16
-    if cin <= 32:
-        return 32
-    return 64
 
 
 def _repack_w3_small(weight, cpt):
@@ -303,6 +296,15 @@
         if key not in d:
             d[key] = fn()
         return d[key]
+
+    def _derived(self, key, fn):
+        held = getattr(self, "_edl_derived", None)
+        if (held is not None and held[0].stamp == _weight_epoch
+                and self.weight.requires_grad):
+            v = held[1].get(key)
+            if v is not None:
+                return v
+        return self._cached(key, fn)
 
     def prefill_derived(self):
         if not self.weight.requires_grad or not self.weight.is_cuda:
@@ -429,7 +431,7 @@
             w3 = self._cached("w3", lambda: _repack_w3(wsrc))
         if cl and mb is not None:
             mode = 0 if self.stride[0] == 1 else 1
-            w3rot = self._cached(
+            w3rot = self._derived(
                 "w3rot" if mode == 0 else "w3s2d",
                 lambda: ext().repack_dgrad_w3(w3, ci, mode))
         elif self.stride[0] == 1:
@@ -462,11 +464,11 @@
         if not x.is_contiguous(memory_format=torch.channels_last):
             x = x.contiguous(memory_format=torch.channels_last)
         cpt = _small_cpt(self.in_channels)
-        w3s = self._cached("w3s", lambda: _repack_w3_small(
+        w3s = self._derived("w3s", lambda: _repack_w3_small(
             self.weight.detach(), cpt))
         w3srot = None
         if self.stride[0] == 1 and x.requires_grad:
-            w3srot = self._cached("w3srot", self._build_w3srot)
+            w3srot = self._derived("w3srot", self._build_w3srot)
         holder = [] if bn_stats else None
         y = _Conv3x3SmallHip.apply(x, self.weight, w3s, w3srot,
                                    self.stride[0], self.out_channels, holder)
@@ -500,7 +502,7 @@
         mb = getattr(self.weight, "_edl_bf16", None)
         if mb is not None:
             w_bf16 = mb.view(co, c)
-            wt_t = self._cached("wt_t", lambda: ext().transpose_pad(
+            wt_t = self._derived("wt_t", lambda: ext().transpose_pad(
                 mb.view(co, c)))
         else:
             w_bf16 = self._cached("w_bf16", lambda: self.weight.detach()
diff --git a/edl_amd/ops/sgd.py b/edl_amd/ops/sgd.py
--- a/edl_amd/ops/sgd.py
+++ b/edl_amd/ops/sgd.py
@@ -16,14 +16,24 @@
         self._buckets = None
         self._use_ext = available() and torch.cuda.is_available()
         self._lr_dev = None
+        self._mirrors = {}
+        self._mirrors_written = set()
         if reducer is not None:
             self.attach(reducer)
 
     def attach(self, reducer):
         self._reducer = reducer
         self._buckets = None
+        self._mirrors = {}
         reducer._attached_opt = self
         return self
+
+    def attach_mirrors(self, pairs):
+        self._mirrors = {flat.data_ptr(): mirror for mirror, flat in pairs}
+
+    def pop_mirrors_written(self):
+        out, self._mirrors_written = self._mirrors_written, set()
+        return out
 
     def set_lr(self, lr):
         for g in self.param_groups:
@@ -67,10 +77,14 @@
             mu = float(momentum)
         if weight_decay is not None:
             wd = float(weight_decay)
+        self._mirrors_written = set()
         for bk in self._materialize():
             if self._use_ext and bk["p"].is_cuda:
+                mirror = self._mirrors.get(bk["p"].data_ptr())
                 ext().fused_sgd(bk["p"], bk["g"], bk["m"], lr, mu, wd,
-                                self.grad_scale, self._lr_dev)
+                                self.grad_scale, self._lr_dev, mirror)
+                if mirror is not None:
+                    self._mirrors_written.add(bk["p"].data_ptr())
             else:
                 g = bk["g"]
                 if self.grad_scale != 1.0:
diff --git a/edl_amd/ops/weight_repack.py b/edl_amd/ops/weight_repack.py
--- /dev/null
+++ b/edl_amd/ops/weight_repack.py
@@ -0,0 +1,120 @@
+from collections import namedtuple
+
+KIND_T, KIND_ROT, KIND_S2D, KIND_SMALL, KIND_SMALLROT = range(5)
+JOB_WORDS = 8
+MAX_JOBS = 1024
+MAX_SOURCES = 16
+SMALL_ELEMS = 2048
+ALIGN = 8
+
+_TAPS_PAD = {16: 12, 32: 10, 64: 9}
+
+Job = namedtuple("Job", "kind key src src_off dst co ci cpt tile_end shape")
+Plan = namedtuple("Plan", "jobs rows arena_numel by_module")
+
+
+def small_cpt(cin):
+    if cin <= 16:
+        return 16
+    if cin <= 32:
+        return 32
+    return 64
+
+
+def job_shape(kind, co, ci, cpt=0):
+    if kind == KIND_T:
+        return (ci, co)
+    if kind in (KIND_ROT, KIND_S2D):
+        return (ci, 9 * co)
+    return (64, _TAPS_PAD[cpt] * cpt)
+
+
+def job_tiles(kind, co, ci, cpt=0):
+    if kind == KIND_T:
+        return (ci // 64) * (co // 64)
+    if kind in (KIND_ROT, KIND_S2D):
+        return 9 * (ci // 64) * (co // 64)
+    out = 64 * _TAPS_PAD[cpt] * cpt
+    return (out + SMALL_ELEMS - 1) // SMALL_ELEMS
+
+
+def conv_jobs(conv, needs_dx=True):
+    co, ci = conv.out_channels, conv.in_channels
+    if (conv.kernel_size == (1, 1) and conv.groups == 1
+            and conv.padding == (0, 0) and conv.bias is None
+            and ci % 64 == 0 and co % 64 == 0):
+        return [(KIND_T, "wt_t", 0)]
+    if (conv._is_dense3x3()
+            and getattr(conv.weight, "_edl_phys_shape", None) is not None):
+        if conv.stride[0] == 1:
+            return [(KIND_ROT, "w3rot", 0)]
+        return [(KIND_S2D, "w3s2d", 0)]
+    if conv._is_small3x3():
+        jobs = [(KIND_SMALL, "w3s", small_cpt(ci))]
+        if conv.stride[0] == 1 and needs_dx:
+            jobs.append((KIND_SMALLROT, "w3srot", small_cpt(co)))
+        return jobs
+    return []
+
+
+def build_plan(bucket_params, convs, first_conv=None, src_aligned=None):
+    where = {}
+    for src, params in enumerate(bucket_params):
+        off = 0
+        for p in params:
+            where[id(p)] = (src, off)
+            off += p.numel()
+    if src_aligned is None:
+        src_aligned = lambda src, off: off % ALIGN == 0
+    jobs, by_module = [], {}
+    dst = tiles = 0
+    for conv in convs:
+        w = conv.weight
+        if not w.requires_grad or id(w) not in where:
+            continue
+        src, off = where[id(w)]
+        co, ci = conv.out_channels, conv.in_channels
+        for kind, key, cpt in conv_jobs(conv, needs_dx=conv is not first_conv):
+            if kind in (KIND_T, KIND_ROT, KIND_S2D) and not src_aligned(
+                    src, off):
+                continue
+            shape = job_shape(kind, co, ci, cpt)
+            tiles += job_tiles(kind, co, ci, cpt)
+            job = Job(kind, key, src, off, dst, co, ci, cpt, tiles, shape)
+            jobs.append(job)
+            by_module.setdefault(id(conv), []).append(job)
+            numel = shape[0] * shape[1]
+            dst += (numel + ALIGN - 1) // ALIGN * ALIGN
+    if len(bucket_params) > MAX_SOURCES or len(jobs) > MAX_JOBS:
+        return Plan([], [], 0, {})
+    rows = [[j.kind, j.src, j.src_off, j.dst, j.co, j.ci, j.tile_end, j.cpt]
+            for j in jobs]
+    return Plan(jobs, rows, dst, by_module)
+
+
+class DerivedArena:
+
+    def __init__(self, plan, mirrors, device):
+        import torch
+
+        self.plan = plan
+        self.mirrors = list(mirrors)
+        self.arena = torch.empty(plan.arena_numel, dtype=torch.bfloat16,
+                                 device=device)
+        self.table_host = torch.tensor(plan.rows, dtype=torch.int32)
+        self.table = self.table_host.to(device)
+        self.stamp = None
+
+    def view(self, job):
+        n = job.shape[0] * job.shape[1]
+        return self.arena[job.dst:job.dst + n].view(*job.shape)
+
+    def views(self, jobs):
+        return {j.key: self.view(j) for j in jobs}
+
+    def refresh(self, epoch):
+        from . import ext
+
+        ext().repack_weights_batched(self.table, self.table_host, self.arena,
+                                     self.mirrors)
+        self.stamp = epoch
diff --git a/edl_amd/train/engine.py b/edl_amd/train/engine.py
--- a/edl_amd/train/engine.py
+++ b/edl_amd/train/engine.py
@@ -239,6 +239,9 @@
 
     def _init_bf16_mirrors(self):
         self._bf16_mirrors = []
+        self._derived_arena = None
+        if hasattr(self.opt, "attach_mirrors"):
+            self.opt.attach_mirrors(())
         if not (self.use_hip_ops and self.device.type == "cuda"):
             return
         for b in self.reducer._buckets:
@@ -251,11 +254,53 @@
             for p in b.params:
                 p._edl_bf16 = _view_like(mirror[off:off + p.numel()], p)
                 off += p.numel()
+        if hasattr(self.opt, "attach_mirrors"):
+            self.opt.attach_mirrors(self._bf16_mirrors)
+        self._init_derived_arena()
         self._refresh_bf16_mirrors()
 
-    def _refresh_bf16_mirrors(self):
+    def _init_derived_arena(self):
+        from ..ops import available
+        from ..ops.conv import Conv2dFast
+        from ..ops.weight_repack import DerivedArena, build_plan
+
+        convs = [m for m in self.model.modules() if isinstance(m, Conv2dFast)]
+        for m in convs:
+            m._edl_derived = None
+        self._derived_arena = None
+        if (not self._bf16_mirrors or not available()
+                or os.environ.get("EDL_DERIVED_BATCH", "1") != "1"
+                or os.environ.get("EDL_PREFILL_DERIVED", "0") == "1"):
+            return
+        mirrors = [m for m, _ in self._bf16_mirrors]
+        flats = {f.data_ptr() for _, f in self._bf16_mirrors}
+        plan = build_plan(
+            [b.params for b in self.reducer._buckets
+             if b.param_flat is not None and b.param_flat.data_ptr() in flats],
+            convs, first_conv=convs[0] if convs else None,
+            src_aligned=lambda src, off:
+                (mirrors[src].data_ptr() + 2 * off) % 16 == 0)
+        if not plan.jobs:
+            if convs:
+                log.warning("no batched weight repack for this model; "
+                            "derived weight layouts are built per conv")
+            return
+        arena = DerivedArena(plan, mirrors, self.device)
+        for m in convs:
+            jobs = plan.by_module.get(id(m))
+            if jobs:
+                m._edl_derived = (arena, arena.views(jobs))
+        self._derived_arena = arena
+
+    def _refresh_bf16_mirrors(self, written=()):
         for mirror, flat in getattr(self, "_bf16_mirrors", ()):
-            mirror.copy_(flat, non_blocking=True)
+            if flat.data_ptr() not in written:
+                mirror.copy_(flat, non_blocking=True)
+        arena = getattr(self, "_derived_arena", None)
+        if arena is not None:
+            from ..ops import conv as conv_ops
+
+            arena.refresh(conv_ops._weight_epoch)
 
     def _build_optimizer(self):
         if self.optimizer != "momentum":
@@ -412,7 +457,10 @@
                     for b in self.reducer._buckets:
                         b.buffer.mul_(scale)
                 self.opt.step()
-            self._refresh_bf16_mirrors()
+            written = ()
+            if hasattr(self.opt, "pop_mirrors_written"):
+                written = self.opt.pop_mirrors_written()
+            self._refresh_bf16_mirrors(written)
         self.global_step += 1
         return loss
 
```

Result: no change. 3863 img/s (median of 6 runs) (+0.7%).
